# LimpBunion22/VIT-FPGA

Hardware: AMD Instinct MI355X
Metric: images/sec ViT-B/16 224x224, batch 512 per GPU (higher is better)
Workload: dtype bf16; 1 GPU; vit_base 224x224x3 inference, 512 images per GPU resident in HBM, random-init weights (seed 0); global_batch=512, per_gpu_batch=512

## Files before the change

vit-fpga_amd/csrc/gemm_epilogue.h:

```cpp
#pragma once

#include "vh_common.h"

namespace vh {

#ifndef VH_EPI_ABL
#define VH_EPI_ABL 0
#endif
#ifndef VH_EPI_NT
#define VH_EPI_NT 1
#endif
template <typename V>
__device__ __forceinline__ void epi_store(V v, V* p) {
    if constexpr (VH_EPI_NT) __builtin_nontemporal_store(v, p);
    else *p = v;
}

struct EpiArgs {
    const float* bias;
    void* out;
    int M, N;
    const float* aux;
    int aux_i;
    const float* stats;
    void* out16;
    float* partials;
    int64_t prow;
    int lead;
};

constexpr bool epi_has_qgelu(int epi) { return epi == VH_EPI_BIAS_QGELU || epi == VH_EPI_LNFOLD_QGELU; }
constexpr bool epi_has_tgelu(int epi) { return epi == VH_EPI_BIAS_TGELU || epi == VH_EPI_LNFOLD_TGELU; }
constexpr bool epi_has_act(int epi) { return epi == VH_EPI_BIAS_GELU || epi == VH_EPI_LNFOLD_GELU || epi_has_qgelu(epi) || epi_has_tgelu(epi); }
constexpr bool epi_is_lnfold(int epi) {
    return epi == VH_EPI_LNFOLD || epi == VH_EPI_LNFOLD_GELU || epi == VH_EPI_LNFOLD_QGELU || epi == VH_EPI_LNFOLD_TGELU;
}
constexpr bool epi_is_16bit(int epi) { return epi == VH_EPI_BIAS || epi == VH_EPI_LNFOLD || epi_has_act(epi); }

__device__ __forceinline__ float gelu_fast(float v) {
    const float u = fabsf(v);
    const float t = __builtin_amdgcn_rcpf(fmaf(0.2316418882f, u, 1.0f));
    float p = fmaf(0.5307027145f, t, -0.7265760135f);
    p = fmaf(p, t, 0.7107068705f);
    p = fmaf(p, t, -0.142248368f);
    p = fmaf(p, t, 0.127414796f);
    p *= t;
    const float h = p * __builtin_amdgcn_exp2f(v * v * -0.72134752044f);
    return fmaf(-u, h, fmaxf(v, 0.f));
}

typedef __attribute__((ext_vector_type(2))) float f32x2;
template <int DEG> struct GeluW;
template <> struct GeluW<9> { static constexpr float a[10] = {1.111100093e-01f, 5.562581867e-02f, 3.875113651e-02f, 7.441916317e-02f, -2.459328771e-01f,
                                                                1.095633626e+00f, -2.419960260e+00f, 3.303298712e+00f, -2.415727854e+00f, 8.016663194e-01f}; };
template <> struct GeluW<8> { static constexpr float a[9] = {1.111119911e-01f, 5.524744466e-02f, 5.048053339e-02f, -6.402773410e-02f, 5.648611188e-01f,
                                                               -1.549515009e+00f, 2.612281084e+00f, -2.240322828e+00f, 8.585962057e-01f}; };
template <> struct GeluW<6> { static constexpr float a[7] = {1.111383960e-01f, 5.238987878e-02f, 9.770081192e-02f, -3.239865899e-01f, 1.061976552e+00f,
                                                               -1.360716462e+00f, 7.577903271e-01f}; };
__device__ __forceinline__ f32x2 pk_fma_clamp01(f32x2 a, f32x2 b, f32x2 c) {
    f32x2 d;
    asm("v_pk_fma_f32 %0, %1, %2, %3 clamp" : "=v"(d) : "v"(a), "v"(b), "v"(c));
    return d;
}
template <int DEG>
__device__ __forceinline__ f32x4 gelu_poly4(f32x4 v) {
    constexpr const float* a = GeluW<DEG>::a;
    f32x2 x[2] = {f32x2{v[0], v[1]}, f32x2{v[2], v[3]}}, w[2], p[2];
#pragma unroll
    for (int h = 0; h < 2; ++h) w[h] = x[h] * x[h];
#pragma unroll
    for (int h = 0; h < 2; ++h) w[h] = pk_fma_clamp01(w[h], f32x2{-4.938271605e-02f, -4.938271605e-02f}, f32x2{1.f, 1.f});
#pragma unroll
    for (int h = 0; h < 2; ++h) p[h] = __builtin_elementwise_fma(w[h], f32x2{a[DEG], a[DEG]}, f32x2{a[DEG - 1], a[DEG - 1]});
#pragma unroll
    for (int k = DEG - 2; k >= 0; --k)
#pragma unroll
        for (int h = 0; h < 2; ++h) p[h] = __builtin_elementwise_fma(p[h], w[h], f32x2{a[k], a[k]});
#pragma unroll
    for (int h = 0; h < 2; ++h) p[h] = pk_fma_clamp01(x[h], p[h], f32x2{0.5f, 0.5f});
#pragma unroll
    for (int h = 0; h < 2; ++h) x[h] = x[h] * p[h];
    return f32x4{x[0][0], x[0][1], x[1][0], x[1][1]};
}
template <typename T> struct GeluDeg { static constexpr int value = 9; };
template <> struct GeluDeg<BF16> { static constexpr int value = 8; };
template <> struct GeluDeg<E4M3> { static constexpr int value = 6; };

__device__ __forceinline__ f32x4 qgelu4(f32x4 v) {
    constexpr float K = -1.702f * 1.44269504088896341f;
    f32x2 x[2] = {f32x2{v[0], v[1]}, f32x2{v[2], v[3]}}, t[2];
// ... 115 lines not shown
                if constexpr (EPI == VH_EPI_BIAS_F32) *p = v;
                else *p = v + addv[ni];
            }
        }
    }
}

#ifndef VH_EPI_PRIO
#define VH_EPI_PRIO 1
#endif
__device__ __forceinline__ void epi_consts_from_lds(const char* sw, int frow, int fq, f32x4 (&bv)[4], f32x4 (&cv)[4], float2 (&lnst)[8]) {
    const uint32_t la = (uint32_t)(uintptr_t)sw + (uint32_t)((fq * 4) * 4), lr = (uint32_t)(uintptr_t)sw + (uint32_t)(frow * 8);
    asm volatile("ds_read_b128 %0, %8 offset:1024\n\tds_read_b128 %1, %8 offset:1088\n\tds_read_b128 %2, %8 offset:1152\n\tds_read_b128 %3, %8 offset:1216\n\t"
                 "ds_read_b128 %4, %8 offset:1280\n\tds_read_b128 %5, %8 offset:1344\n\tds_read_b128 %6, %8 offset:1408\n\tds_read_b128 %7, %8 offset:1472"
                 : "=&v"(bv[0]), "=&v"(bv[1]), "=&v"(bv[2]), "=&v"(bv[3]), "=&v"(cv[0]), "=&v"(cv[1]), "=&v"(cv[2]), "=&v"(cv[3]) : "v"(la));
    asm volatile("ds_read_b64 %0, %8\n\tds_read_b64 %1, %8 offset:128\n\tds_read_b64 %2, %8 offset:256\n\tds_read_b64 %3, %8 offset:384\n\t"
                 "ds_read_b64 %4, %8 offset:512\n\tds_read_b64 %5, %8 offset:640\n\tds_read_b64 %6, %8 offset:768\n\tds_read_b64 %7, %8 offset:896\n\t"
                 "s_waitcnt lgkmcnt(0)"
                 : "=&v"(lnst[0]), "=&v"(lnst[1]), "=&v"(lnst[2]), "=&v"(lnst[3]), "=&v"(lnst[4]), "=&v"(lnst[5]), "=&v"(lnst[6]), "=&v"(lnst[7]) : "v"(lr));
    asm volatile("" : "+v"(bv[0]), "+v"(bv[1]), "+v"(bv[2]), "+v"(bv[3]), "+v"(cv[0]), "+v"(cv[1]), "+v"(cv[2]), "+v"(cv[3]));
}

template <typename T, int EPI, int MI, int NI, int SMI = MI, bool MFULL = false, bool OTILED = false>
__device__ __forceinline__ void gemm_epilogue_staged(const f32x4 (&acc)[MI][NI], const EpiArgs& e, int m_w, int n_w,
                                                     int lane, char* sw, int prio_grp = -1, bool cpre = false) {
    static_assert(NI == 4, "staged epilogue assumes a 64-column wave tile");
    static_assert(MI % SMI == 0 && SMI % 2 == 0, "slice must divide the wave tile");
    using elem = typename T::elem;
    const int M = e.M, N = e.N;
    const int frow = lane & 15, fq = lane >> 4;
    f32x4 bv[NI], cv[NI];
    float2 lnst[epi_is_lnfold(EPI) ? MI : 1];
    auto consts_from_global = [&]() {
#pragma unroll
        for (int ni = 0; ni < NI; ++ni) {
            bv[ni] = *(const f32x4*)(e.bias + n_w + ni * 16 + fq * 4);
            if constexpr (epi_is_lnfold(EPI)) cv[ni] = *(const f32x4*)(e.aux + n_w + ni * 16 + fq * 4);
            else cv[ni] = f32x4{0.f, 0.f, 0.f, 0.f};
        }
        if constexpr (epi_is_lnfold(EPI)) {
#pragma unroll
            for (int mi = 0; mi < MI; ++mi) {
                int m = m_w + mi * 16 + frow;
                if constexpr (!MFULL) m = m < M ? m : M - 1;
                lnst[mi] = *(const float2*)(e.stats + 2 * (int64_t)m);
            }
        }
    };
    if constexpr (epi_is_lnfold(EPI) && MI == 8) {
        if (cpre) epi_consts_from_lds(sw, frow, fq, bv, cv, lnst);
        else consts_from_global();
    } else {
        consts_from_global();
    }

    if constexpr (epi_is_16bit(EPI) && (VH_EPI_ABL & 64)) {
#pragma unroll
        for (int mi = 0; mi < MI; ++mi)
#pragma unroll
            for (int ni = 0; ni < NI; ++ni) asm volatile("" :: "v"(acc[mi][ni]));
    } else if constexpr (epi_is_16bit(EPI) && epi_has_act(EPI) && MFULL && OTILED) {
        char* const obase = (char*)e.out + ((int64_t)(m_w >> 4) * (N >> 3) + (n_w >> 3) + (fq & 1) * 2 + (fq >> 1)) * 256 + frow * 16;
#pragma unroll
        for (int mi = 0; mi < MI; ++mi) {
            if constexpr (VH_EPI_PRIO == 1) {
                if (prio_grp >= 0 && (mi & 1) == 0) {
                    if (((mi >> 1) + prio_grp) & 1) __builtin_amdgcn_s_setprio(1);
                    else __builtin_amdgcn_s_setprio(0);
                }
            }
            float rstd = 0.f, mr = 0.f;
            if constexpr (epi_is_lnfold(EPI)) { rstd = lnst[mi].y; mr = lnst[mi].x * lnst[mi].y; }
#pragma unroll
            for (int j = 0; j < NI / 2; ++j) {
                const f32x4 v0 = epi_value16<EPI, T>(acc[mi][2 * j], bv[2 * j], cv[2 * j], mr, rstd);
                const f32x4 v1 = epi_value16<EPI, T>(acc[mi][2 * j + 1], bv[2 * j + 1], cv[2 * j + 1], mr, rstd);
                const u32x2 p0 = __builtin_bit_cast(u32x2, pack4<T>(v0[0], v0[1], v0[2], v0[3]));
                const u32x2 p1 = __builtin_bit_cast(u32x2, pack4<T>(v1[0], v1[1], v1[2], v1[3]));
                const auto sx = __builtin_amdgcn_permlane16_swap(p0[0], p1[0], false, false);
                const auto sy = __builtin_amdgcn_permlane16_swap(p0[1], p1[1], false, false);
                epi_store(u32x4{sx[0], sy[0], sx[1], sy[1]}, (u32x4*)(obase + (int64_t)mi * (N >> 3) * 256 + j * 1024));
            }
        }
        if constexpr (VH_EPI_PRIO == 1) { if (prio_grp >= 0) __builtin_amdgcn_s_setprio(0); }
    } else if constexpr (epi_is_16bit(EPI)) {
        const int rr = lane >> 3, pc = lane & 7;
#pragma unroll
        for (int h = 0; h < MI / SMI; ++h) {
            if constexpr (VH_EPI_PRIO == 1) {
                if (prio_grp >= 0) {
                    if ((h + prio_grp) & 1) __builtin_amdgcn_s_setprio(1);
                    else __builtin_amdgcn_s_setprio(0);
                }
            }
#pragma unroll
            for (int mi = 0; mi < SMI; ++mi) {
                if constexpr (VH_EPI_PRIO == 2) {
                    if (prio_grp >= 0) {
                        if ((h * SMI + mi + prio_grp) & 1) __builtin_amdgcn_s_setprio(1);
                        else __builtin_amdgcn_s_setprio(0);
                    }
                }
                const int r = mi * 16 + frow;
                float rstd = 0.f, mr = 0.f;
                if constexpr (epi_is_lnfold(EPI)) {
                    const float2 st = lnst[h * SMI + mi];
// ... 344 lines not shown
```

vit-fpga_amd/csrc/kernels_attn.hip:

```cpp
#include <type_traits>

#include "attn_common.h"

namespace vh {

template <typename T, typename TO = T>
__global__ void __launch_bounds__(1024, 4)
attention_kernel(const typename T::elem* __restrict__ qkv, typename TO::elem* __restrict__ out,
                 int tokens, int heads, int slabs, int ntiles) {
    using elem = typename T::elem;
    using vec8 = typename T::vec8;
    using vec4 = typename T::vec4;
    extern __shared__ __attribute__((aligned(16))) char smem[];
    const int kv_bytes = ntiles * 4096;

    const int lane = threadIdx.x & 63;
    const int wave = __builtin_amdgcn_readfirstlane(threadIdx.x >> 6);
    const int nw = blockDim.x >> 6;
    const int l31 = lane & 31, hl = lane >> 5;
    const int D = heads * 64;
    const int64_t ld = 3 * (int64_t)D;

    const int lr = lane >> 3, pc = lane & 7;
    const int ngroups = ntiles * 4;
// ... 116 lines not shown
        f32x16 s_cur = qk(0);
        for (int kt = 0; kt + 1 < ntiles; ++kt) {
            const VFrag vfr = load_v(kt);
            const f32x16 s_nxt = qk(kt + 1);
            softmax_pv(kt, s_cur, vfr, std::false_type{});
            s_cur = s_nxt;
        }
        {
            const VFrag vfr = load_v(ntiles - 1);
            softmax_pv(ntiles - 1, s_cur, vfr, std::true_type{});
        }

        const float ltot = cross_half_sum(lsum);
        const float inv = 1.0f / ltot;
        const int q = q0 + l31;
        if (q < tokens) {
            typename TO::elem* op = out + ((int64_t)b * tokens + q) * D + h * 64 + 4 * hl;
#pragma unroll
            for (int rg = 0; rg < 4; ++rg) {
                *(typename TO::vec4*)(op + 8 * rg) = pack4<TO>(o0[4 * rg] * inv, o0[4 * rg + 1] * inv, o0[4 * rg + 2] * inv, o0[4 * rg + 3] * inv);
                *(typename TO::vec4*)(op + 32 + 8 * rg) = pack4<TO>(o1[4 * rg] * inv, o1[4 * rg + 1] * inv, o1[4 * rg + 2] * inv, o1[4 * rg + 3] * inv);
            }
        }
    }
}

#ifndef VH_ATTN_ABL
#define VH_ATTN_ABL 0
#endif
__device__ __forceinline__ void ring_dma16(const void* base, uint32_t lane_off, uint32_t lds_addr) {
    asm_lds_dma16(base, lane_off, lds_addr);
}
#ifdef VH_DIAG_STAMPS
__device__ unsigned long long g_attn_diag[1024 * 16 * 16];
__device__ __forceinline__ unsigned long long attn_rt() {
    unsigned long long t;
    asm volatile("s_memrealtime %0\n\ts_waitcnt lgkmcnt(0)" : "=s"(t)::"memory");
    return t;
}
__device__ __forceinline__ unsigned long long attn_ct() {
    unsigned long long t;
    asm volatile("s_memtime %0\n\ts_waitcnt lgkmcnt(0)" : "=s"(t)::"memory");
    return t;
}
#define VH_ATT_T(i) do { __builtin_amdgcn_sched_barrier(0); const unsigned long long n_ = attn_ct(); ph_[i] += n_ - last_; last_ = n_; __builtin_amdgcn_sched_barrier(0); } while (0)
#else
#define VH_ATT_T(i) do { } while (0)
#endif
__device__ __forceinline__ void ring_wait_vm(int n) { wait_vm<40>(n); }
__device__ __forceinline__ void ring_wait_dma() {
    asm volatile("s_waitcnt vmcnt(0)" ::: "memory");
}

template <typename T, typename TO = T, bool QS = false, bool OTILE = false, bool IHM = false>
__global__ void __launch_bounds__(1024, 4)
attention_ring_kernel(const typename T::elem* __restrict__ qkv, typename TO::elem* __restrict__ out,
                      int tokens, int heads, int slabs, int ntiles, int nitems, unsigned int* __restrict__ ticket,
                      unsigned int heads_rcp, int64_t hm_rows) {
    using elem = typename T::elem;
    using vec8 = typename T::vec8;
    using vec4 = typename T::vec4;
    extern __shared__ __attribute__((aligned(16))) char smem[];
    const int G = (tokens + 7) >> 3, G2 = (G + 1) & ~1;
    const int kv_bytes = QS ? G * 1024 : ntiles * 4096;
    const int q_off = kv_bytes + (QS ? G2 * 1024 : kv_bytes);
    const uint32_t lds0 = (uint32_t)(uintptr_t)smem;

    const int lane = threadIdx.x & 63;
    const int wave = __builtin_amdgcn_readfirstlane(threadIdx.x >> 6);
    const int nw = blockDim.x >> 6;
    const int l31 = lane & 31, hl = lane >> 5;
    const int D = heads * 64;
    const int64_t ld = IHM ? 64 : 3 * (int64_t)D;
    const uint32_t koff2 = IHM ? (uint32_t)(hm_rows * D * 2) : (uint32_t)(D * 2);
    auto head_base = [&](int b, int h) {
        if constexpr (IHM) return qkv + ((int64_t)h * hm_rows + (int64_t)b * tokens) * 64;
        else return qkv + (int64_t)b * tokens * ld + h * 64;
    };

    auto kv_base = [&](int item) {
        if (QS) {
            const int b = (heads == 1 ? item : (int)__umulhi((unsigned)item, heads_rcp)), h = item - b * heads;
            return head_base(b, h);
        }
        const int bh = item / slabs;
        const int b = bh / heads, h = bh - b * heads;
        return head_base(b, h);
    };
    auto issue_tile = [&](const elem* base, int t) {
        int ln = lane;
        asm volatile("" : "+v"(ln));
        const int lr_ = ln >> 3, pc_ = ln & 7;
        const int g = 4 * t + wave;
        const int gk = QS && g >= G ? G - 1 : g, gv = QS && g >= G2 ? G2 - 1 : g;
        const int rowk = gk * 8 + lr_, rowv = gv * 8 + lr_;
        const int rk = rowk < tokens ? rowk : tokens - 1;
        const int rv = rowv < tokens ? rowv : tokens - 1;
        const int ck = pc_ ^ ((rowk >> 1) & 7);
        const int cv = pc_ ^ (((rowv >> 1) & 1) << 2);
        const uint32_t ok = (uint32_t)(rk * (int)ld + ck * 8) * 2u + koff2;
        const uint32_t ov = (uint32_t)(rv * (int)ld + cv * 8) * 2u + 2u * koff2;
        ring_dma16(base, ok, lds0 + gk * 1024);
        ring_dma16(base, ov, lds0 + kv_bytes + gv * 1024);
    };
    auto issue_q = [&](const elem* base) {
        int ln = lane;
        asm volatile("" : "+v"(ln));
        const int lr_ = ln >> 3, pc_ = ln & 7;
        for (int j = 0; j < nw; ++j) {
            const int g = 4 * j + wave;
            const int row = g * 8 + lr_;
            const int rsrc = row < tokens ? row : tokens - 1;
            const int ck = pc_ ^ ((row >> 1) & 7);
            ring_dma16(base, (uint32_t)(rsrc * (int)ld + ck * 8) * 2u, lds0 + q_off + g * 1024);
        }
    };
    auto load_q = [&](int item, vec8 (&qf)[4]) {
        const int bh = item / slabs, slab = item - bh * slabs;
        const int b = bh / heads, h = bh - b * heads;
        int qrow = (slab * nw + wave) * 32 + l31;
        qrow = qrow < tokens ? qrow : tokens - 1;
        const elem* qp = head_base(b, h) + (int64_t)qrow * ld + 8 * hl;
        asm volatile("global_load_dwordx4 %0, %4, off\n\tglobal_load_dwordx4 %1, %4, off offset:32\n\t"
                     "global_load_dwordx4 %2, %4, off offset:64\n\tglobal_load_dwordx4 %3, %4, off offset:96"
                     : "=&v"(qf[0]), "=&v"(qf[1]), "=&v"(qf[2]), "=&v"(qf[3]) : "v"(qp) : "memory");
    };

    const int kswz = (l31 >> 1) & 7;
    const int g4 = lane >> 4, i16 = lane & 15, tq = i16 >> 2, tp = i16 & 3;
    const int vrow0 = 4 * (g4 >> 1) + tq;
    const int vcolb = (16 * (g4 & 1) + 4 * tp) * 2;
    const int k0 = l31 * 128 + ((hl ^ kswz) << 4);
    const int vx = ((vrow0 >> 1) & 1) << 6;
    const int v0 = kv_bytes + vrow0 * 128 + (vcolb ^ vx);

    const int stride = (int)gridDim.x;
    int item = blockIdx.x * slabs;
    const elem* cbase = kv_base(item);
    vec8 qf[4];
    if (wave < 4) {
        if (QS) issue_q(cbase);
        for (int t = 0; t < ntiles; ++t) issue_tile(cbase, t);
    }
    if (!QS) load_q(item, qf);
    bool first = true;
    constexpr int NST = 4;
    const int w_top = 2 * (ntiles - 2) + NST, w_t1 = 2 * (ntiles - 3) + NST + 2, w_mid = 2 * ntiles + nw - 4 + NST, w_last = nw + 2 + 2 * (ntiles - 3);
    bool stored = false;

#ifdef VH_DIAG_STAMPS
    const unsigned long long rt0_ = attn_rt();
    unsigned int dbg_[3] = {0xffffffffu, 0xffffffffu, 0xffffffffu};
    int dbg_n_ = 0;
    unsigned long long ph_[10] = {0, 0, 0, 0, 0, 0, 0, 0, 0, 0}, last_ = attn_ct();
#endif
    const bool dyn = QS && ticket != nullptr && nw >= 5;
    const int tk_off = q_off + 4 * nw * 1024;
    unsigned int tkv = 0;
    while (true) {
        const int slab_now = QS ? 0 : item - (item / slabs) * slabs;
        const bool last_slab = QS || slab_now + 1 == slabs;
        int next = QS ? item + stride : (last_slab ? (item / slabs + stride) * slabs : item + 1);
        if (QS && dyn && !first) {
            if (wave == nw - 1) {
                if (stored) asm volatile("s_waitcnt vmcnt(%0)" :: "n"(NST) : "memory");
                else asm volatile("s_waitcnt vmcnt(0)" ::: "memory");
                asm volatile("" : "+v"(tkv));
                if (lane == 0) *(volatile unsigned int __attribute__((address_space(3)))*)(uintptr_t)(lds0 + tk_off) = 2u * (unsigned)stride + tkv;
            }
        }
        const int b = QS ? (heads == 1 ? item : (int)__umulhi((unsigned)item, heads_rcp)) : (item / slabs) / heads;
        const int slab = slab_now;
        const int h = (QS ? item : item / slabs) - b * heads;
        const int q0 = (slab * nw + wave) * 32;

        VH_ATT_T(7);
        if (QS) {
            ring_wait_vm(first ? 0 : w_top);
        } else {
            if (first || !stored) asm volatile("s_waitcnt vmcnt(0)" ::: "memory");
            else asm volatile("s_waitcnt vmcnt(%0)" :: "n"(NST) : "memory");
            asm volatile("" : "+v"(qf[0]), "+v"(qf[1]), "+v"(qf[2]), "+v"(qf[3]));
        }
        VH_ATT_T(0);
        ring_barrier();
        VH_ATT_T(1);
        if (QS && dyn && !first) next = __builtin_amdgcn_readfirstlane(*(volatile const int __attribute__((address_space(3)))*)(uintptr_t)(lds0 + tk_off));
#if defined(VH_DIAG_STAMPS) && defined(VH_ATTN_TKDBG)
        if (QS && dyn && !first) { if (dbg_n_ < 3) dbg_[dbg_n_++] = (unsigned)next; next = item + stride; }
#endif
        const bool has_next = (unsigned)next < (unsigned)nitems;
        const bool refill = has_next && last_slab;
        const elem* nbase = kv_base(has_next ? next : item);
        if (QS && dyn && has_next && wave == nw - 1 && lane == 0) {
            asm_atomic_add_ret_issue(ticket, 1u, tkv);
        }
        if (!(VH_ATTN_ABL & 2) && !first && slab == 0 && wave < 4) issue_tile(cbase, ntiles - 1);
        if (QS) {
            int qa = q_off + wave * 4096 + k0;
            if constexpr (!std::is_same<T, TO>::value) {
                int ln = lane;
                asm volatile("" : "+v"(ln));
                const int r31 = ln & 31;
                qa = q_off + wave * 4096 + r31 * 128 + ((((ln >> 5)) ^ ((r31 >> 1) & 7)) << 4);
            }
#pragma unroll
            for (int ks = 0; ks < 4; ++ks) qf[ks] = *(const vec8*)(smem + (qa ^ (ks << 5)));
        }

        f32x16 o0, o1;
#pragma unroll
        for (int r = 0; r < 16; ++r) { o0[r] = 0.f; o1[r] = 0.f; }
        float negm = 0.f;
        float lsum = 0.f;

        auto qk = [&](int kt, float init) {
            int ka = k0 + kt * 4096;
            if constexpr (!std::is_same<T, TO>::value) asm volatile("" : "+v"(ka));
            vec8 kf[4];
#pragma unroll
            for (int ks = 0; ks < 4; ++ks) {
                if (VH_ATTN_ABL & 32) kf[ks] = qf[ks]; else if (VH_ATTN_ABL & 128) kf[ks] = *(const vec8*)(smem + ((ka ^ (ks << 5)) & 0x3ff0)); else
                kf[ks] = *(const vec8*)(smem + (ka ^ (ks << 5)));
            }
            __builtin_amdgcn_sched_barrier(0);
            typedef float f32x2 __attribute__((ext_vector_type(2)));
            typedef float f32x8 __attribute__((ext_vector_type(8)));
            const f32x2 i2 = {init, init};
            f32x2 p[8];
#pragma unroll
            for (int i = 0; i < 8; ++i) asm volatile("v_mov_b64 %0, %1" : "=v"(p[i]) : "v"(i2));
            const f32x4 q0 = __builtin_shufflevector(p[0], p[1], 0, 1, 2, 3), q1 = __builtin_shufflevector(p[2], p[3], 0, 1, 2, 3);
            const f32x4 q2 = __builtin_shufflevector(p[4], p[5], 0, 1, 2, 3), q3 = __builtin_shufflevector(p[6], p[7], 0, 1, 2, 3);
            const f32x8 h0 = __builtin_shufflevector(q0, q1, 0, 1, 2, 3, 4, 5, 6, 7), h1 = __builtin_shufflevector(q2, q3, 0, 1, 2, 3, 4, 5, 6, 7);
            f32x16 s = __builtin_shufflevector(h0, h1, 0, 1, 2, 3, 4, 5, 6, 7, 8, 9, 10, 11, 12, 13, 14, 15);
#pragma unroll
            for (int ks = 0; ks < 4; ++ks) {
                if (VH_ATTN_ABL & 16) s[ks] += (float)kf[ks][0] * (float)qf[ks][0];
                else s = T::mfma32(kf[ks], qf[ks], s);
            }
            return s;
        };
        struct VFrag { vec8 f[2][2]; };
        auto load_v = [&](int kt) {
            VFrag v;
            if (VH_ATTN_ABL & 32) { for (int ks = 0; ks < 2; ++ks) { v.f[ks][0] = qf[ks]; v.f[ks][1] = qf[ks + 2]; } return v; }
            const char* p0 = smem + (v0 + kt * 4096);
            const char* p1 = smem + ((v0 + kt * 4096) ^ 64);
#pragma unroll
            for (int ks = 0; ks < 2; ++ks) {
                const vec4 a0 = T::tr_read(p0 + ks * 2048), c0 = T::tr_read(p0 + ks * 2048 + 1024);
                const vec4 a1 = T::tr_read(p1 + ks * 2048), c1 = T::tr_read(p1 + ks * 2048 + 1024);
#pragma unroll
                for (int j = 0; j < 4; ++j) { v.f[ks][0][j] = a0[j]; v.f[ks][0][4 + j] = c0[j]; v.f[ks][1][j] = a1[j]; v.f[ks][1][4 + j] = c1[j]; }
            }
            return v;
        };
        auto softmax_pv = [&](int kt, f32x16& s, const VFrag& vfr, auto first_c, auto tail_c) {
            constexpr bool FIRST = decltype(first_c)::value, TAIL = decltype(tail_c)::value;
            int ng = 4;
            if constexpr (TAIL) {
                const int valid = tokens - kt * 32;
                ng = (valid + 7) >> 3;
#pragma unroll
                for (int g = 0; g < 4; ++g)
                    if (g < ng) {
#pragma unroll
                        for (int j = 0; j < 4; ++j)
                            if (8 * g + j + 4 * hl >= valid) s[4 * g + j] = -INFINITY;
                    }
            }
            float mx = -INFINITY;
#pragma unroll
            for (int g = 0; g < 4; ++g)
                if (!TAIL || g < ng) {
#pragma unroll
// ... 96 lines not shown
                    }
                }
            } else {
                const int64_t mrow = (int64_t)b * tokens + (q < tokens ? q : tokens - 1);
                typename TO::elem* const op = OTILE ? out + ((mrow >> 4) * (D >> 4) + h * 4) * 256 + (mrow & 15) * 16 + 8 * hl
                                                    : out + mrow * D + h * 64 + 8 * hl;
#pragma unroll
                for (int db = 0; db < 2; ++db) {
                    const f32x16& o = db ? o1 : o0;
#pragma unroll
                    for (int rg = 0; rg < 4; rg += 2) {
                        const uint32_t ga = pack4<TO>(o[4 * rg] * inv, o[4 * rg + 1] * inv, o[4 * rg + 2] * inv, o[4 * rg + 3] * inv);
                        const uint32_t gb = pack4<TO>(o[4 * rg + 4] * inv, o[4 * rg + 5] * inv, o[4 * rg + 6] * inv, o[4 * rg + 7] * inv);
                        const auto sx = __builtin_amdgcn_permlane32_swap(ga, gb, false, false);
                        if (q < tokens) *(u32x2*)(op + (OTILE ? (2 * db + (rg >> 1)) * 256 : 32 * db + 8 * rg)) = u32x2{sx[0], sx[1]};
                    }
                }
            }
        }
        VH_ATT_T(9);
        if (!has_next) break;
        stored = q0 < tokens;
        item = next;
        cbase = nbase;
        first = false;
    }
#ifdef VH_DIAG_STAMPS
    VH_ATT_T(7);
    if (lane == 0 && blockIdx.x < 1024) {
#pragma unroll
        for (int i = 0; i < 10; ++i) g_attn_diag[((size_t)blockIdx.x * 16 + wave) * 16 + i] = ph_[i];
        unsigned int hw;
        asm volatile("s_getreg_b32 %0, hwreg(HW_REG_HW_ID)" : "=s"(hw));
        unsigned int xcc;
        asm volatile("s_getreg_b32 %0, hwreg(HW_REG_XCC_ID)" : "=s"(xcc));
        g_attn_diag[((size_t)blockIdx.x * 16 + wave) * 16 + 10] = rt0_;
        g_attn_diag[((size_t)blockIdx.x * 16 + wave) * 16 + 11] = attn_rt();
        g_attn_diag[((size_t)blockIdx.x * 16 + wave) * 16 + 12] = ((unsigned long long)xcc << 32) | hw;
        for (int i = 0; i < 3; ++i) g_attn_diag[((size_t)blockIdx.x * 16 + wave) * 16 + 13 + i] = dbg_[i];
    }
#endif
}

#ifdef VH_DIAG_STAMPS
extern "C" int vh_diag_attn_read(unsigned long long* host, int n_words) {
    return (int)hipMemcpyFromSymbol(host, HIP_SYMBOL(g_attn_diag), (size_t)n_words * 8);
}
#endif

size_t attention_lds_bytes(int tokens) { return (size_t)((tokens + 31) / 32) * 8192; }

enum class AttnForm { NONE, ONE_SHOT, RING, RING_QS };
struct AttnPlan { AttnForm form; int slabs, nw; size_t lds; };
static AttnPlan attn_plan(int tokens, bool out_tiled, bool in_head_major) {
    constexpr int kMaxWaves = 16;
    const int ntiles = (tokens + 31) / 32;
    const int slabs = (ntiles + kMaxWaves - 1) / kMaxWaves, nw = (ntiles + slabs - 1) / slabs;
    const size_t one = attention_lds_bytes(tokens);
    if (one > 160 * 1024) return {AttnForm::NONE, slabs, nw, 0};
    const int G = (tokens + 7) / 8, G2 = (G + 1) & ~1;
    const size_t qs_lds = (size_t)(G + G2 + 4 * nw) * 1024 + 16;
    if (slabs == 1 && nw >= 4 && 2 * qs_lds <= 160 * 1024) return {AttnForm::RING_QS, slabs, nw, qs_lds};
    if (ntiles >= 3 && nw >= 4) return {AttnForm::RING, slabs, nw, one};
    if (out_tiled || in_head_major) return {AttnForm::NONE, slabs, nw, 0};
    return {AttnForm::ONE_SHOT, slabs, nw, one};
}
bool attention_tiled_applies(int batch, int tokens, int heads) {
    (void)batch;
    return attn_plan(tokens, true, false).form != AttnForm::NONE && heads % 2 == 0;
}

template <typename T, typename TO = T, bool OTILE = false, bool IHM = false>
static hipError_t launch_attn_t(const void* qkv, int batch, int tokens, int heads, void* out, unsigned int* ticket, hipStream_t s, bool tk_zeroed,
                                int64_t hm_rows = 0) {
    const AttnPlan p = attn_plan(tokens, OTILE, IHM);
    if (p.form == AttnForm::NONE) return hipErrorInvalidValue;
    const int ntiles = (tokens + 31) / 32, slabs = p.slabs, nw = p.nw;
    const int nitems = batch * heads * slabs;
    const int num_cu = device_num_cu();
    if (!num_cu) return hipErrorUnknown;
    if (p.form == AttnForm::RING_QS) {
        auto k = attention_ring_kernel<T, TO, true, OTILE, IHM>;
        static LdsDone lds_done;
        if (hipError_t e = ensure_dynamic_lds((const void*)k, p.lds, lds_done); e != hipSuccess) return e;
        const int grid = nitems < 2 * num_cu ? nitems : 2 * num_cu;
        unsigned int* tk = nw >= 5 && nitems > 2 * grid ? ticket : nullptr;
        if (tk && !tk_zeroed) { if (hipError_t e = hipMemsetAsync(tk, 0, sizeof(unsigned int), s); e != hipSuccess) return e; }
        const unsigned int heads_rcp = (unsigned int)(((1ull << 32) + (unsigned)heads - 1) / (unsigned)heads);
        hipLaunchKernelGGL(k, dim3(grid), dim3(nw * 64), p.lds, s, (const typename T::elem*)qkv, (typename TO::elem*)out,
                           tokens, heads, slabs, ntiles, nitems, tk, heads_rcp, hm_rows);
        return hipGetLastError();
    }
    if (p.form == AttnForm::RING) {
        auto k = attention_ring_kernel<T, TO, false, OTILE, IHM>;
        static LdsDone lds_done;
        if (hipError_t e = ensure_dynamic_lds((const void*)k, p.lds, lds_done); e != hipSuccess) return e;
        const int per_cu = (int)(160 * 1024 / p.lds);
        int grid = num_cu * (per_cu < 1 ? 1 : (per_cu > 2 ? 2 : per_cu));
        if (grid > batch * heads) grid = batch * heads;
        hipLaunchKernelGGL(k, dim3(grid), dim3(nw * 64), p.lds, s, (const typename T::elem*)qkv, (typename TO::elem*)out,
                           tokens, heads, slabs, ntiles, nitems, (unsigned int*)nullptr, 0u, hm_rows);
        return hipGetLastError();
    }
    if constexpr (OTILE || IHM) return hipErrorInvalidValue;
    else {
        auto k = attention_kernel<T, TO>;
        static LdsDone lds_done;
        if (hipError_t e = ensure_dynamic_lds((const void*)k, p.lds, lds_done); e != hipSuccess) return e;
        hipLaunchKernelGGL(k, dim3(nitems), dim3(nw * 64), p.lds, s, (const typename T::elem*)qkv, (typename TO::elem*)out,
                           tokens, heads, slabs, ntiles);
        return hipGetLastError();
    }
}

template <typename T>
__global__ void __launch_bounds__(256)
attention_cls_kernel(const typename T::elem* __restrict__ qkv, typename T::elem* __restrict__ out, int batch, int tokens, int heads) {
    using elem = typename T::elem;
    using vec8 = typename T::vec8;
    constexpr int MAXT = 1024;
    __shared__ float sc[4][MAXT];
    const int lane = threadIdx.x & 63, wv = threadIdx.x >> 6;
    const int item = blockIdx.x * 4 + wv;
    if (item >= batch * heads) return;
    const int b = item / heads, h = item - b * heads;
    const int D = heads * 64;
    const int64_t ld = 3 * (int64_t)D;
    const elem* const base = qkv + (int64_t)b * tokens * ld + h * 64;
    const int g = lane >> 3, c = lane & 7;
    float q[8];
    {
        const vec8 v = *(const vec8*)(base + c * 8);
#pragma unroll
        for (int j = 0; j < 8; ++j) q[j] = (float)v[j];
    }
    float mx = -INFINITY;
    constexpr int U = 4;
    for (int t0 = 0; t0 < tokens; t0 += 8 * U) {
        vec8 v[U];
#pragma unroll
        for (int u = 0; u < U; ++u) {
            const int t = t0 + 8 * u + g;
            v[u] = *(const vec8*)(base + (t < tokens ? t : tokens - 1) * ld + D + c * 8);
        }
#pragma unroll
        for (int u = 0; u < U; ++u) {
            const int t = t0 + 8 * u + g;
// ... 10 lines not shown
#pragma unroll
    for (int o = 32; o > 0; o >>= 1) mx = fmaxf(mx, __shfl_xor(mx, o));
    __builtin_amdgcn_s_waitcnt(0xC07F);
    float sum = 0.f;
    for (int t = lane; t < tokens; t += 64) {
        const float p = __builtin_amdgcn_exp2f(sc[wv][t] - mx);
        sc[wv][t] = p;
        sum += p;
    }
#pragma unroll
    for (int o = 32; o > 0; o >>= 1) sum += __shfl_xor(sum, o);
    __builtin_amdgcn_s_waitcnt(0xC07F);
    float acc[8] = {0.f, 0.f, 0.f, 0.f, 0.f, 0.f, 0.f, 0.f};
    for (int t0 = 0; t0 < tokens; t0 += 8 * U) {
        vec8 v[U];
#pragma unroll
        for (int u = 0; u < U; ++u) {
            const int t = t0 + 8 * u + g;
            v[u] = *(const vec8*)(base + (t < tokens ? t : tokens - 1) * ld + 2 * D + c * 8);
        }
#pragma unroll
        for (int u = 0; u < U; ++u) {
            const int t = t0 + 8 * u + g;
            const float p = t < tokens ? sc[wv][t] : 0.f;
#pragma unroll
            for (int j = 0; j < 8; ++j) acc[j] = fmaf(p, (float)v[u][j], acc[j]);
        }
    }
#pragma unroll
    for (int j = 0; j < 8; ++j) {
        acc[j] += __shfl_xor(acc[j], 8); acc[j] += __shfl_xor(acc[j], 16); acc[j] += __shfl_xor(acc[j], 32);
    }
    if (g == 0) {
        const float r = 1.0f / sum;
        vec8 o;
#pragma unroll
        for (int j = 0; j < 8; ++j) o[j] = (elem)(acc[j] * r);
        *(vec8*)(out + (int64_t)b * D + h * 64 + c * 8) = o;
    }
}
hipError_t launch_attention_cls(const void* qkv16, int batch, int tokens, int heads, void* out16, int dtype, hipStream_t s) {
    if (batch <= 0 || tokens <= 0 || tokens > 1024 || heads <= 0) return hipErrorInvalidValue;
    const dim3 grid((unsigned)((batch * heads + 3) / 4));
    if (dtype == VH_DTYPE_BF16)
        hipLaunchKernelGGL(attention_cls_kernel<BF16>, grid, dim3(256), 0, s, (const BF16::elem*)qkv16, (BF16::elem*)out16, batch, tokens, heads);
    else if (dtype == VH_DTYPE_FP16)
        hipLaunchKernelGGL(attention_cls_kernel<FP16>, grid, dim3(256), 0, s, (const FP16::elem*)qkv16, (FP16::elem*)out16, batch, tokens, heads);
    else
        return hipErrorInvalidValue;
    return hipGetLastError();
}

hipError_t launch_attention(const void* qkv16, int batch, int tokens, int heads, void* out16, int dtype,
                            unsigned int* ticket, hipStream_t s, bool ticket_zeroed, bool out_tiled, int64_t in_hm_rows) {
    if (batch <= 0 || tokens <= 0 || heads <= 0) return hipErrorInvalidValue;
    if (in_hm_rows) {
        if (!out_tiled || in_hm_rows < (int64_t)batch * tokens || in_hm_rows * heads * 64 * 4 >= (1ll << 32)) return hipErrorInvalidValue;
        if (!attention_tiled_applies(batch, tokens, heads)) return hipErrorInvalidValue;
        if (dtype == VH_DTYPE_FP8) return launch_attn_t<BF16, E4M3, true, true>(qkv16, batch, tokens, heads, out16, ticket, s, ticket_zeroed, in_hm_rows);
        return dtype == VH_DTYPE_BF16 ? launch_attn_t<BF16, BF16, true, true>(qkv16, batch, tokens, heads, out16, ticket, s, ticket_zeroed, in_hm_rows)
                                      : launch_attn_t<FP16, FP16, true, true>(qkv16, batch, tokens, heads, out16, ticket, s, ticket_zeroed, in_hm_rows);
    }
    if (out_tiled) {
        if (!attention_tiled_applies(batch, tokens, heads)) return hipErrorInvalidValue;
        if (dtype == VH_DTYPE_FP8) return launch_attn_t<BF16, E4M3, true>(qkv16, batch, tokens, heads, out16, ticket, s, ticket_zeroed);
        return dtype == VH_DTYPE_BF16 ? launch_attn_t<BF16, BF16, true>(qkv16, batch, tokens, heads, out16, ticket, s, ticket_zeroed)
                                      : launch_attn_t<FP16, FP16, true>(qkv16, batch, tokens, heads, out16, ticket, s, ticket_zeroed);
    }
    if (attention_lds_bytes(tokens) > 160 * 1024) return launch_attention_hd(qkv16, batch, tokens, heads, 64, out16, dtype, s);
    if (dtype == VH_DTYPE_FP8) return launch_attn_t<BF16, E4M3>(qkv16, batch, tokens, heads, out16, ticket, s, ticket_zeroed);
    return dtype == VH_DTYPE_BF16 ? launch_attn_t<BF16>(qkv16, batch, tokens, heads, out16, ticket, s, ticket_zeroed)
                                  : launch_attn_t<FP16>(qkv16, batch, tokens, heads, out16, ticket, s, ticket_zeroed);
}

}
```

vit-fpga_amd/csrc/kernels_gemm.hip:

```cpp
#include <cstdio>
#include <cstdlib>

#include "gemm_epilogue.h"
#include "vh_kernels.h"

namespace vh {

template <typename T, int BM, int BN, int WM, int WN, int EPI>
__global__ void __launch_bounds__(WM* WN * 64)
gemm_nt_kernel(const typename T::elem* __restrict__ A, const typename T::elem* __restrict__ W,
               const float* __restrict__ bias, void* __restrict__ outp, int M, int N, int K,
               const float* __restrict__ aux, int aux_i, int tiles_m, int tiles_n, const float* __restrict__ stats,
               void* __restrict__ out16, float* __restrict__ partials, int64_t prow, int lead) {
    using elem = typename T::elem;
    using vec8 = typename T::vec8;
    constexpr int NW = WM * WN;
    constexpr int BK = 64;
    constexpr int ROWS = BM + BN;
    constexpr int STAGE_BYTES = ROWS * 128;
    constexpr int GROUPS_A = BM / 8;
    constexpr int GROUPS = ROWS / 8;
    constexpr int LOADS = GROUPS / NW;
    constexpr int LOADS_A = GROUPS_A / NW;
    constexpr int TM = BM / WM, TN = BN / WN;
// ... 134 lines not shown
    const int64_t t256 = ((M + 255) / 256) * ((N + 255) / 256);
    return t256 >= min_tiles ? gemm_pp_variant(epilogue) : 1;
}

bool gemm_tiled_applies(int64_t M, int N, int K, int dtype) {
    const bool f8 = dtype == VH_DTYPE_FP8;
    const int kt = f8 ? 128 : 64;
    return M > 0 && M % 256 == 0 && N % 256 == 0 && K % kt == 0 && K / kt >= 4 &&
           (f8 ? gemm_pp_variant(VH_EPI_BIAS) : gemm_pick_variant(M, N, VH_EPI_BIAS)) == 6;
}

const char* gemm_check(const GemmArgs& g) {
    const int epi = g.epilogue;
    const bool f8 = g.dtype == VH_DTYPE_FP8;
    const bool act = epi_has_act(epi), fold = epi_is_lnfold(epi), resid = epi == VH_EPI_RESID_LN || epi == VH_EPI_RESID_SPLIT;
    if (f8) {
        if (g.variant != 0 && g.variant != 5 && g.variant != 6 && g.variant != 7) return "gemm_fp8: variant must be 0, 5, 6 or 7";
        if (!g.a || !g.w || !g.wscale || !g.bias || !g.out) return "gemm_fp8: null pointer";
        if (g.M <= 0 || g.N <= 0 || g.K <= 0 || g.K % 128 || g.N % 4) return "gemm_fp8: need K % 128 == 0 and N % 4 == 0";
        if (g.M > 0x7FFFFFFF / 2) return "gemm_fp8: M too large";
        if (!fold && !resid && !act && epi != VH_EPI_BIAS && epi != VH_EPI_BIAS_RESID && epi != VH_EPI_BIAS_F32)
            return "gemm_fp8: epilogue not available";
        if (fold && (!g.aux || !g.stats)) return "gemm_fp8: LNFOLD needs c and stats";
        if (resid && (!g.out16 || !g.partials)) return "gemm_fp8: RESID_* needs out16 and partials";
        if ((resid || (fold && act)) && g.N % 256) return "gemm_fp8: N % 256 != 0";
    } else {
        if (g.M <= 0 || g.N <= 0 || g.K <= 0) return "gemm: empty shape";
        if (g.K % 64) return "gemm: K must be a multiple of 64";
        if (g.N % 4) return "gemm: N must be a multiple of 4";
        if (g.M > 0x7fffffff) return "gemm: M too large";
        if (epi < 0 || epi > VH_EPI_LNFOLD_TGELU || epi == VH_EPI_LNFOLD_QGELU + 1) return "gemm: unknown epilogue";
        if (fold && (!g.stats || !g.aux)) return "gemm: LNFOLD needs stats and c (aux)";
        if (resid && (!g.out16 || !g.partials || g.N % 256)) return "gemm: RESID_LN / RESID_SPLIT need out16, partials and N % 256 == 0";
        if (epi == VH_EPI_PATCH && (!g.aux || g.aux_i <= 0)) return "gemm: EPI_PATCH needs pos-emb and patches/image";
        if ((epi == VH_EPI_PATCH || epi == VH_EPI_PATCH_SPLIT) && (g.lead < 0 || g.lead > 1 + VH_MAX_REGISTERS)) return "gemm: EPI_PATCH* lead rows outside 0..17";
        if (epi == VH_EPI_PATCH_SPLIT && (!g.aux || g.aux_i <= 0 || !g.out16 || !g.partials || g.N % 256 || g.prow < 0))
            return "gemm: EPI_PATCH_SPLIT needs pos-emb, patches/image, the lo plane, partials and N % 256 == 0";
        if (g.dtype != VH_DTYPE_BF16 && g.dtype != VH_DTYPE_FP16) return "gemm: dtype";
        if (g.variant < 0 || g.variant > 7) return "gemm: variant";
        if (g.variant == 3 || g.variant == 4) return "gemm: variants 3/4 (BK=32 pipeline) were removed";
        if (!g.a || !g.w || !g.bias || !g.out) return "gemm: null pointer";
    }
    if (g.out_tiled || g.ab_tiled) {
        if (g.out_tiled && g.ab_tiled) return "gemm_layout: out_tiled and ab_tiled exclude each other";
        if (g.variant != 6) return "gemm_layout: the tiled layouts exist in the persistent form only (variant 6)";
        if (g.tile_begin || g.tile_count) return "gemm_layout: a tile range excludes the tiled layouts";
        if (g.M % 256 || g.N % 256) return "gemm_layout: the tiled layouts need M % 256 == 0 and N % 256 == 0";
        const bool four = fold && !(f8 && act);
        if (g.K / (f8 ? 128 : 64) < (four ? 4 : 2))
            return four ? "gemm_layout: the tiled layouts need at least 4 K-tiles with this epilogue"
                        : "gemm_layout: the tiled layouts need at least 2 K-tiles with this epilogue";
        if (g.out_tiled && !(act || epi == VH_EPI_LNFOLD || (!f8 && epi == VH_EPI_BIAS)))
            return "gemm_layout: out_tiled goes with the activation epilogues (tiled) or LNFOLD / 16-bit BIAS (head-major)";
        if (g.ab_tiled && !(epi == VH_EPI_RESID_SPLIT || (!f8 && epi == VH_EPI_BIAS))) return "gemm_layout: ab_tiled goes with RESID_SPLIT or 16-bit BIAS";
    }
    if (g.tile_begin < 0 || g.tile_count < 0) return "gemm_layout: negative tile range";
    if (g.tile_begin || g.tile_count) {
        if (g.variant != 5 && g.variant != 7) return "gemm_layout: tile ranges exist in variants 5 and 7 only";
        if (!g.tile_count) return "gemm_layout: tile_begin != 0 needs tile_count > 0";
        const int64_t tiles = ((g.M + 255) / 256) * ((g.N + 255) / 256);
        if ((int64_t)g.tile_begin + g.tile_count > tiles) {
            static thread_local char text[64];
            snprintf(text, sizeof text, "gemm_layout: tile range beyond the %lld tiles", (long long)tiles);
            return text;
        }
    }
    return nullptr;
}

hipError_t launch_gemm_fp8(const GemmArgs& g, hipStream_t s);

hipError_t launch_gemm(const GemmArgs& g, hipStream_t s) {
    if (gemm_check(g)) return hipErrorInvalidValue;
    if (g.dtype == VH_DTYPE_FP8) return launch_gemm_fp8(g, s);
    const int variant = g.variant ? g.variant : gemm_pick_variant(g.M, g.N, g.epilogue);
    return g.dtype == VH_DTYPE_BF16 ? launch_epi<BF16>(g, variant, s) : launch_epi<FP16>(g, variant, s);
}

}
```

vit-fpga_amd/csrc/kernels_gemm5.hip:

```cpp
#include <cstdlib>
#include <type_traits>

#include "gemm_epilogue.h"
#include "vh_kernels.h"

#ifndef VH_PP_SMI
#define VH_PP_SMI 2
#endif

namespace vh {

#ifndef VH_MAIN_ABL
#define VH_MAIN_ABL 0
#endif
#ifndef VH_PP_CPRE
#define VH_PP_CPRE 1
#endif
constexpr int kAblHalf = (VH_MAIN_ABL & 64) ? 1 : 0;
constexpr int kWPieces = kAblHalf ? 2 : 4;
#ifdef VH_DIAG_STAMPS
#ifndef VH_DIAG_KT
#define VH_DIAG_KT -1
#endif
#ifndef VH_DIAG_REC_IT
// ... 412 lines not shown
    if (env >= 0) return env > 0 && env < tiles_n ? env : 0;
    if (tiles_n < 6) return 0;
    if (tiles_n % 4 == 0) return 4;
    if (tiles_n % 3 == 0) return 3;
    return 4;
}

#ifdef VH_DIAG_STAMPS
struct DiagRec { int64_t M; int N, K, epi, f8, grid, variant; };
static unsigned long long* g_diag_buf = nullptr;
static int g_diag_slots = 0, g_diag_max_wgs = 0;
static long long g_diag_count = 0;
static DiagRec g_diag_rec[1024];
static unsigned long long* diag_next(const GemmArgs& g, int epi, bool f8, int grid, int variant) {
    if (!g_diag_buf || grid > g_diag_max_wgs) return nullptr;
    const int slot = (int)(g_diag_count % g_diag_slots);
    g_diag_rec[slot] = DiagRec{g.M, g.N, g.K, epi, f8 ? 1 : 0, grid, variant};
    ++g_diag_count;
    return g_diag_buf + (size_t)slot * g_diag_max_wgs * 128;
}
#define VH_STAMP_ARG(g, epi, f8, grid, variant) , diag_next(g, epi, f8, grid, variant)
#else
#define VH_STAMP_ARG(g, epi, f8, grid, variant)
#endif

template <typename T, int EPI, bool F8, bool PERSIST, int AST, bool OT = false, bool AT = false>
static hipError_t launch_pp_one(const GemmArgs& g, int grid, int tiles_m, int tiles_n, hipStream_t s) {
    constexpr size_t lds = (AST == 3 || PERSIST) ? 163840 : 131072;
    auto k = gemm_nt_pp_kernel<T, EPI, PERSIST, F8, AST, OT, AT>;
    static LdsDone lds_done;
    if (hipError_t e = ensure_dynamic_lds((const void*)k, lds, lds_done); e != hipSuccess) return e;
    hipLaunchKernelGGL(k, dim3(grid), dim3(512), lds, s, g.a, g.w, g.bias, g.out, (int)g.M, g.N, g.K, g.aux, g.aux_i, tiles_m,
                       tiles_n, g.stats, g.out16, g.partials, PERSIST ? 0 : g.tile_begin, (g.tile_count || g.tile_begin) ? 0 : gemm_super_columns(tiles_n),
                       F8 ? g.wscale : (const float*)nullptr, gemm_prow(g), g.lead
                       VH_STAMP_ARG(g, EPI, F8, grid, PERSIST ? 6 : (AST == 3 ? 7 : 5)));
    return hipGetLastError();
}

template <typename T, int EPI, bool F8>
static hipError_t launch_pp(const GemmArgs& g, int mode, hipStream_t s) {
    if constexpr (EPI == VH_EPI_PATCH) { if (mode == 1) mode = 0; }
    const int tiles_m = (int)((g.M + 255) / 256), tiles_n = (g.N + 255) / 256;
    const int ntiles = g.tile_count > 0 ? g.tile_count : tiles_m * tiles_n;
    if (mode == 2) return launch_pp_one<T, EPI, F8, false, 3>(g, ntiles, tiles_m, tiles_n, s);
    if constexpr (EPI != VH_EPI_PATCH) {
        const int full_m = (int)(g.M / 256);
        const int nk = g.K / (F8 ? 128 : 64);
        if (mode == 1 && (g.N % 256 != 0 || full_m == 0 || nk < (pp_uses_cpre<EPI, F8>() ? 4 : 2))) mode = 0;
        if (mode == 1 && full_m != tiles_m && g.variant != 6) mode = 0;
        if (mode == 1) {
            const int num_cu = device_num_cu();
            if (!num_cu) return hipErrorUnknown;
            const int nfull = full_m * tiles_n, grid = nfull < num_cu ? nfull : num_cu;
            if constexpr (epi_has_act(EPI) || EPI == VH_EPI_LNFOLD || (!F8 && EPI == VH_EPI_BIAS)) {
                if (g.out_tiled) return launch_pp_one<T, EPI, F8, true, 2, true, false>(g, grid, full_m, tiles_n, s);
            }
            if constexpr (F8 ? EPI == VH_EPI_RESID_SPLIT : (EPI == VH_EPI_RESID_SPLIT || EPI == VH_EPI_BIAS)) {
                if (g.ab_tiled) return launch_pp_one<T, EPI, F8, true, 2, false, true>(g, grid, full_m, tiles_n, s);
            }
            if (hipError_t e = launch_pp_one<T, EPI, F8, true, 2>(g, grid, full_m, tiles_n, s); e != hipSuccess) return e;
            if (full_m == tiles_m) return hipSuccess;
            GemmArgs tail = g;
            tail.tile_begin = nfull;
            tail.tile_count = tiles_n;
            return launch_pp_one<T, EPI, F8, false, 2>(tail, tiles_n, tiles_m, tiles_n, s);
        }
    }
    return launch_pp_one<T, EPI, F8, false, 2>(g, ntiles, tiles_m, tiles_n, s);
}

template <typename T, int EPI>
hipError_t launch_gemm_pingpong(const GemmArgs& g, int mode, hipStream_t s) {
    return launch_pp<T, EPI, false>(g, mode, s);
}

#define VH_INST(T)                                                                                     \
    template hipError_t launch_gemm_pingpong<T, VH_EPI_BIAS>(const GemmArgs&, int, hipStream_t);       \
    template hipError_t launch_gemm_pingpong<T, VH_EPI_BIAS_GELU>(const GemmArgs&, int, hipStream_t);  \
    template hipError_t launch_gemm_pingpong<T, VH_EPI_BIAS_RESID>(const GemmArgs&, int, hipStream_t); \
    template hipError_t launch_gemm_pingpong<T, VH_EPI_BIAS_F32>(const GemmArgs&, int, hipStream_t);   \
    template hipError_t launch_gemm_pingpong<T, VH_EPI_PATCH>(const GemmArgs&, int, hipStream_t);       \
    template hipError_t launch_gemm_pingpong<T, VH_EPI_LNFOLD>(const GemmArgs&, int, hipStream_t);      \
    template hipError_t launch_gemm_pingpong<T, VH_EPI_LNFOLD_GELU>(const GemmArgs&, int, hipStream_t); \
    template hipError_t launch_gemm_pingpong<T, VH_EPI_RESID_LN>(const GemmArgs&, int, hipStream_t);   \
    template hipError_t launch_gemm_pingpong<T, VH_EPI_RESID_SPLIT>(const GemmArgs&, int, hipStream_t); \
    template hipError_t launch_gemm_pingpong<T, VH_EPI_PATCH_SPLIT>(const GemmArgs&, int, hipStream_t); \
    template hipError_t launch_gemm_pingpong<T, VH_EPI_BIAS_QGELU>(const GemmArgs&, int, hipStream_t);  \
    template hipError_t launch_gemm_pingpong<T, VH_EPI_LNFOLD_QGELU>(const GemmArgs&, int, hipStream_t); \
    template hipError_t launch_gemm_pingpong<T, VH_EPI_BIAS_TGELU>(const GemmArgs&, int, hipStream_t);  \
    template hipError_t launch_gemm_pingpong<T, VH_EPI_LNFOLD_TGELU>(const GemmArgs&, int, hipStream_t);
VH_INST(BF16)
VH_INST(FP16)

hipError_t launch_gemm_fp8(const GemmArgs& g, hipStream_t s) {
    const int v = g.variant ? g.variant : gemm_pp_variant(g.epilogue);
    const int mode = v == 7 ? 2 : (v == 6 ? 1 : 0);
    switch (g.epilogue) {
        case VH_EPI_BIAS: return launch_pp<BF16, VH_EPI_BIAS, true>(g, mode, s);
        case VH_EPI_BIAS_GELU: return launch_pp<BF16, VH_EPI_BIAS_GELU, true>(g, mode, s);
        case VH_EPI_BIAS_QGELU: return launch_pp<BF16, VH_EPI_BIAS_QGELU, true>(g, mode, s);
        case VH_EPI_BIAS_TGELU: return launch_pp<BF16, VH_EPI_BIAS_TGELU, true>(g, mode, s);
        case VH_EPI_BIAS_RESID: return launch_pp<BF16, VH_EPI_BIAS_RESID, true>(g, mode, s);
        case VH_EPI_BIAS_F32: return launch_pp<BF16, VH_EPI_BIAS_F32, true>(g, mode, s);
        case VH_EPI_LNFOLD: return launch_pp<BF16, VH_EPI_LNFOLD, true>(g, mode, s);
        case VH_EPI_LNFOLD_GELU: return launch_pp<BF16, VH_EPI_LNFOLD_GELU, true>(g, mode, s);
        case VH_EPI_LNFOLD_QGELU: return launch_pp<BF16, VH_EPI_LNFOLD_QGELU, true>(g, mode, s);
// ... 33 lines not shown
```

vit-fpga_amd/csrc/vh_kernels.h:

```cpp
#pragma once

#include <atomic>
#include <cstdlib>
#include <vector>

#include "vh_common.h"

namespace vh {

struct GemmArgs {
    const void* a;
    const void* w;
    const float* bias;
    void* out;
    int64_t M;
    int N, K;
    int epilogue;
    const float* aux;
    int aux_i;
    int dtype;
    int variant;
    const float* stats = nullptr;
    void* out16 = nullptr;
    float* partials = nullptr;
    const float* wscale = nullptr;
    int tile_begin = 0, tile_count = 0;
    int64_t prow = 0;
    int out_tiled = 0, ab_tiled = 0;
    int lead = 1;
};
bool gemm_tiled_applies(int64_t M, int N, int K, int dtype);
hipError_t launch_cast_tiled_w(const float* w, int rows, int cols, void* w16, int dtype, hipStream_t stream);
hipError_t launch_tile_bytes(const void* w8, int rows, int cols, void* out, hipStream_t stream);

inline int64_t gemm_prow(const GemmArgs& g) {
    if (g.epilogue != VH_EPI_PATCH_SPLIT) return g.M;
    return g.prow > 0 ? g.prow : (g.M / g.aux_i) * (int64_t)(g.aux_i + g.lead);
}

hipError_t launch_gemm(const GemmArgs& g, hipStream_t stream);
const char* gemm_check(const GemmArgs& g);
int gemm_pick_variant(int64_t M, int N, int epilogue);
int gemm_pp_variant(int epilogue);

hipError_t launch_layernorm(const float* x, int64_t rows, int dim, int64_t row_stride,
                            const float* gamma, const float* beta, float eps, void* out16,
                            int dtype, hipStream_t stream);
hipError_t launch_head_f32(const float* y, const float* w, const float* bias, float* out, int batch, int classes, int dim,
                           hipStream_t stream);
hipError_t launch_head_f32_groups(const float* y, int64_t ldy, int64_t y_step, const float* w, const float* bias, float* out, int64_t ldo,
                                  const float* add, int batch, int classes, int dim, int groups, hipStream_t stream);
hipError_t launch_act_f32(float* x, int64_t n, int act, hipStream_t stream);
constexpr float kAttnQScale = 0.125f * 1.4426950408889634f;
hipError_t launch_attention(const void* qkv16, int batch, int tokens, int heads, void* out16,
                            int dtype, unsigned int* ticket, hipStream_t stream, bool ticket_zeroed = false, bool out_tiled = false,
                            int64_t in_hm_rows = 0);
bool attention_tiled_applies(int batch, int tokens, int heads);
hipError_t launch_attention_cls(const void* qkv16, int batch, int tokens, int heads, void* out16, int dtype, hipStream_t stream);
size_t attention_lds_bytes(int tokens);
constexpr int kAttnStreamMaxTokens = 4097;
constexpr int kAttnHdMaxWidth = 2048;
bool attention_hd_supported(int head_dim);
hipError_t launch_attention_hd(const void* qkv16, int batch, int tokens, int heads, int head_dim, void* out16, int dtype,
                               hipStream_t stream);
constexpr int kAttnMapsMaxQueries = 17;
const char* attention_probs_check(int64_t in_hm_rows, int batch, int tokens, int heads, int head_dim, int Q, int dtype);
hipError_t launch_attention_probs(const void* qkv16, int64_t in_hm_rows, int batch, int tokens, int heads, int head_dim, int Q, int dtype,
                                  float* probs, hipStream_t stream);
const char* rope_check(const void* qkv16, int dtype, int batch, int tokens, int heads, int head_dim, int lead, int64_t hm_rows,
                       const float* cos_t, const float* sin_t);
hipError_t launch_rope(void* qkv16, int dtype, int batch, int tokens, int heads, int head_dim, int lead, int64_t hm_rows, const float* cos_t,
                       const float* sin_t, hipStream_t stream);
const char* attention_readout_check(int batch, int heads, int Q, int tokens, int lead, int elem, int keys);
hipError_t launch_attention_readout(const float* store, int batch, int heads, int Q, int tokens, int lead, int elem, int keys, void* probs_out,
                                    void* mean_out, hipStream_t stream);
inline float attention_q_scale(int head_dim) {
    return head_dim == 64 ? kAttnQScale : (float)(1.4426950408889634 / __builtin_sqrt((double)head_dim));
}
hipError_t launch_im2col(const float* in_nhwc, int batch, int image, int patch, int channels, int kpad,
                         void* out16, int dtype, hipStream_t stream);
constexpr int kMaxChannels = 64;
hipError_t launch_im2col_u8(const uint8_t* in_nhwc, int batch, int image, int patch, int channels, int kpad,
                            const float* scale, const float* shift, void* out16, int dtype, hipStream_t stream);
hipError_t launch_im2col_tensor(const void* in, int elem, int layout, int batch, int image, int patch, int channels, int kpad,
                                const float* scale, const float* shift, void* out16, int dtype, hipStream_t stream);
constexpr int kResizeMaxTaps = 65, kResizeMaxScale = 32, kResizeMaxSide = 8192;
constexpr int kResizeLdsFloats = 16384;
constexpr int kResizeFrameWords = 16;
int resize_axis_table(int n_in, double lo, double hi, int n_out, int32_t* first, int32_t* count, float* weights, int max_taps);
const char* resize_plan_build(const vh_frame* desc, int batch, int channels, int S, size_t nbytes, bool base_aligned4,
                              std::vector<uint32_t>* words, int* max_tiles);
hipError_t launch_resize_u8(const uint8_t* frames, const uint32_t* plan_dev, int batch, int channels, int S, int max_tiles,
                            uint8_t* out_u8, hipStream_t stream);
constexpr int kResizeNv12FrameWords = 24;
int resize_axis_table_over(int n_in, double lo, double hi, double over, int n_out, int32_t* first, int32_t* count, float* weights,
                           int max_taps);
const char* resize_plan_build_nv12(const vh_frame_nv12* desc, int batch, int S, size_t nbytes, unsigned base_mod4, int chroma_site,
                                   int sample_bytes, std::vector<uint32_t>* words, int* max_tiles);
int yuv_matrix(int standard, int full_range, float m[12]);
const char* resize_plan_build_yuv(const vh_frame_yuv* desc, int batch, int S, size_t nbytes, bool base_even, int chroma_site, int sample_bytes,
                                  std::vector<uint32_t>* words, int* max_tiles);
int yuv_matrix16(int standard, int full_range, int bits, int msb_aligned, float m[12]);
hipError_t launch_resize_yuv_any(bool planar, bool wide, const uint8_t* frames, const uint32_t* plan_dev, int batch, int S, int max_tiles,
                                 const float* m12_host, uint8_t* out_u8, hipStream_t stream);
const char* resize_plan_build_yuy2(const vh_frame_yuy2* desc, int batch, int S, size_t nbytes, unsigned base_mod8, int chroma_site,
                                   int sample_bytes, std::vector<uint32_t>* words, int* max_tiles);
hipError_t launch_resize_yuy2(bool wide, const uint8_t* frames, const uint32_t* plan_dev, int batch, int S, int max_tiles,
                              const float* m12_host, uint8_t* out_u8, hipStream_t stream);
const char* resize_plan_build_bgra(const vh_frame_bgra* desc, int batch, int S, size_t nbytes, unsigned base_mod8, int sample_bytes,
                                   std::vector<uint32_t>* words, int* max_tiles);
// ... 115 lines not shown
```

vit-fpga_amd/csrc/vithip_api.hip:

```cpp
#include <dlfcn.h>

#include <chrono>
#include <cmath>
#include <condition_variable>
#include <cstdarg>
#include <cstdio>
#include <cstdlib>
#include <cstring>
#include <functional>
#include <memory>
#include <mutex>
#include <string>
#include <thread>
#include <vector>

#include "vh_kernels.h"

using namespace vh;

namespace {

thread_local std::string g_err;

int fail(std::string* ctx_err, int code, const char* fmt, ...) {
// ... 164 lines not shown
}

struct ImgIn {
    const void* p;
    int kind = VH_ELEM_F32;
    int layout = VH_LAYOUT_NHWC;
    bool u8() const { return kind == VH_ELEM_U8; }
    bool nhwc_f32() const { return kind == VH_ELEM_F32 && layout == VH_LAYOUT_NHWC; }
    size_t elem() const { return kind == VH_ELEM_F32 ? 4 : kind == VH_ELEM_U8 ? 1 : 2; }
    ImgIn skip(size_t elements) const { return ImgIn{(const char*)p + elements * elem(), kind, layout}; }
    bool operator==(const ImgIn& o) const { return p == o.p && kind == o.kind && layout == o.layout; }
};
constexpr int kU8 = VH_ELEM_U8;

struct ActSet {
    char* base = nullptr;
    unsigned int* tickets = nullptr;
    float* x = nullptr;
    void* xn16 = nullptr;
    void* xlo16 = nullptr;
    void* qkv16 = nullptr;
    void* att16 = nullptr;
    void* h16 = nullptr;
    void* col16 = nullptr;
    float* clsn32 = nullptr;
    float* pool32 = nullptr;
    float* stats = nullptr;
    float* partials = nullptr;
    float *mapz32 = nullptr, *maph32 = nullptr, *mapa32 = nullptr;
};
struct ActSetLayout { size_t x, xn, qkv, att, h, col, cls, pool, st, pt, xlo, tk, mz, mh, ma, bytes; };

struct vh_ctx {
    vh_config cfg;
    int device;
    Layout L;
    hipStream_t stream = nullptr;
    static constexpr int kMaxStreams = 4;
    hipStream_t xstream[kMaxStreams - 1] = {nullptr, nullptr, nullptr};
    hipEvent_t ev_fork = nullptr, ev_join[kMaxStreams - 1] = {nullptr, nullptr, nullptr};
    int nstreams = 1;
    hipEvent_t ev0 = nullptr, ev1 = nullptr;
    bool weights_ready = false;
    int run_layers = -1;
    char* blob = nullptr;
    float* params = nullptr;
    char* w16 = nullptr;
    void* wp16 = nullptr;
    std::vector<void*> wqkv16, wo16, w1_16, w2_16;
    std::vector<void*> w2t_16, wot_16;
    bool h_tiled = false;
    bool att_tiled = true;
    bool qkv_hm = true;
    bool weights_ready_tiled = false;
    float* bqkv = nullptr;
    bool fp8 = false;
    int dt16 = VH_DTYPE_BF16;
    std::vector<float*> sqkv, so, s1, s2;
    bool ln_fold = false;
    float* fold_cd = nullptr;
    bool split = false;
    bool cls_tail = false;
    int head_dim = 64;
    float q_scale = kAttnQScale;
    bool ln_fold_cfg = false, split_cfg = false;
    unsigned int* guard_dev = nullptr;
    float* guard_host = nullptr;
    float guard_thresh = 0.5f;
    bool guard_auto = false, guard_tripped = false;
    char* arena = nullptr;
    ActSet act[2];
    ActSetLayout act_layout{};
    int last_set = 0;
    hipStream_t stream2 = nullptr;
    hipEvent_t ev_fork2 = nullptr, ev_join2 = nullptr, ev_head[2] = {nullptr, nullptr};
    int inflight_max = 2, ring_flip = 0;
    bool s2_open = false;
    float* in_dev = nullptr;
    float in_scale[kMaxChannels], in_shift[kMaxChannels];
    float* logits_dev = nullptr;
    uint8_t* rz_u8 = nullptr;
    uint32_t *rz_plan_dev = nullptr, *rz_plan_host = nullptr;
    size_t rz_plan_dev_cap = 0, rz_plan_host_cap = 0;
    uint8_t* rz_frames = nullptr;
    size_t rz_frames_cap = 0;
    std::vector<uint32_t> rz_words;
    struct FrameColour { float m[12]; int site = VH_CHROMA_LEFT; };
    FrameColour colour[2];
    int64_t last_us = 0;
    bool timed = false;
    int last_batch = 0;
    int feat_layers[VH_MAX_FEATURE_LAYERS] = {0}, feat_n = 0;
    char* feat_store = nullptr;
    size_t feat_slot = 0;
    int cap_layers[VH_MAX_FEATURE_LAYERS] = {0}, cap_n = 0, cap_nl = -1, cap_form = VH_FEAT_FORM_F32;
    int attn_layers[VH_MAX_ATTENTION_LAYERS] = {0}, attn_n = 0, attn_q = 0, attn_mode = VH_ATTN_Q_CLS;
    char* attn_store = nullptr;
    size_t attn_slot = 0;
    int acap_layers[VH_MAX_ATTENTION_LAYERS] = {0}, acap_n = 0, acap_nl = -1;
    struct RingSlot {
        float *h_in = nullptr, *h_out = nullptr, *d_in = nullptr, *d_out = nullptr;
        hipEvent_t in_done = nullptr, fwd_done = nullptr, out_done = nullptr;
        int batch = 0;
        uint32_t* h_plan = nullptr;
        size_t plan_cap = 0;
    };
    std::vector<RingSlot> ring;
    enum RingKind { RING_F32, RING_U8, RING_FRAMES, RING_TENSOR };
    RingKind ring_kind = RING_F32;
    int ring_elem = VH_ELEM_F32, ring_layout = VH_LAYOUT_NHWC;
    size_t ring_slot_bytes = 0;
    hipStream_t copy_in = nullptr, copy_out = nullptr;
    int ring_batch = 0, ring_wr = 0, ring_rd = 0, ring_used = 0;
    bool last_h_tiled = false;
    bool last_qkv_hm = false;
    int num_cu = 256;
    bool use_graph = false;
    struct GraphEntry { ImgIn in; float* out; int batch; hipGraph_t graph; hipGraphExec_t exec; };
    std::vector<GraphEntry> graphs;
    std::vector<int> graph_warm;
    int timing_stage = -1;
    std::vector<hipEvent_t> tev;
    size_t tev_used = 0;
    bool step_timing = false;
    std::vector<hipEvent_t> sev;
    size_t sev_used = 0;
    std::string err;
};

struct vh_filter {
    int device, height, width, kind;
    struct Slot {
        uint8_t *h_in = nullptr, *h_out = nullptr, *d_in = nullptr, *d_out = nullptr;
        hipEvent_t in_done = nullptr, k_done = nullptr, out_done = nullptr;
    };
    std::vector<Slot> slot;
    hipStream_t copy_in = nullptr, compute = nullptr, copy_out = nullptr;
    int wr = 0, rd = 0, used = 0;
    std::string err;
};

struct vh_mlp {
    int device, n_ins, n_layers, activation;
    std::vector<int> npl;
    size_t n_params = 0, n_neurons = 0;
    int widest = 0, max_vec = 0;
    hipStream_t stream = nullptr;
    float *params = nullptr, *bias = nullptr, *buf0 = nullptr, *buf1 = nullptr;
    bool loaded = false;
    int64_t last_us = 0;
    int n_sets = 0;
    float *set_ins = nullptr, *set_outs = nullptr, *tz = nullptr, *ta = nullptr, *td = nullptr, *terr = nullptr;
    int64_t last_gradient_us = 0;
    std::string err;
};

namespace {

size_t align_up(size_t v, size_t a) { return (v + a - 1) / a * a; }

int set_device(std::string* err, int device) {
    int n = 0;
    hipError_t e = hipGetDeviceCount(&n);
    if (e != hipSuccess || n <= 0) return fail(err, VH_ERR_NO_DEVICE, "no HIP device visible (%s)", hipGetErrorString(e));
    if (device < 0 || device >= n) return fail(err, VH_ERR_INVALID, "device %d out of range (0..%d)", device, n - 1);
    HIPCHK(err, hipSetDevice(device));
    return VH_OK;
}
// ... 233 lines not shown
    const bool pre_ln = (f.flags & VH_FLAG_PRE_LN) != 0;
    const bool quick = (f.flags & VH_FLAG_QUICK_GELU) != 0, tanh_gelu = (f.flags & VH_FLAG_TANH_GELU) != 0;
    const int epi_fc1 = quick ? VH_EPI_LNFOLD_QGELU : tanh_gelu ? VH_EPI_LNFOLD_TGELU : VH_EPI_LNFOLD_GELU;
    const int epi_fc1_plain = quick ? VH_EPI_BIAS_QGELU : tanh_gelu ? VH_EPI_BIAS_TGELU : VH_EPI_BIAS_GELU;
    const bool patch_split = c->split && !c->fp8 && nl > 0 && !pre_ln;
    if ((rc = tmark(ST_IM2COL))) return rc;
    if (in.layout == VH_LAYOUT_NHWC && in.u8())
        HIPCHK(&c->err, launch_im2col_u8((const uint8_t*)in.p, batch, f.image_size, f.patch_size, f.channels, L.KPA, c->in_scale, c->in_shift,
                                         col16, dt16, s));
    else if (in.nhwc_f32())
        HIPCHK(&c->err, launch_im2col((const float*)in.p, batch, f.image_size, f.patch_size, f.channels, L.KPA, col16, dt16, s));
    else
        HIPCHK(&c->err, launch_im2col_tensor(in.p, in.kind, in.layout, batch, f.image_size, f.patch_size, f.channels, L.KPA, c->in_scale,
                                             c->in_shift, col16, dt16, s));
    if ((rc = tmark(ST_IM2COL))) return rc;
    if ((rc = mark(ST_IM2COL))) return rc;
    if (patch_split) {
        GemmArgs g = gemm_args(dt16, col16, c->wp16, P + L.patch_b, xn16, (int64_t)batch * L.NP, D, L.KPA, VH_EPI_PATCH_SPLIT, pos_p, L.NP);
        g.out16 = xlo16;
        g.prow = rows_g;
        g.lead = L.lead;
        if ((rc = stage(ST_PATCH, [&] { return launch_gemm(g, s); }))) return rc;
        if ((rc = stage(ST_CLS, [&] {
                 return launch_lead_rows_split(xn16, xlo16, partials_p, rows_g, cls_p, pos_p, P + L.reg, L.lead, batch, T, D, dt16, s);
             })))
            return rc;
        HIPCHK(&c->err, launch_finalize_stats(partials_p, D / 64, rows_g, D, f.ln_eps, stats_p, s, rows, c->guard_dev, amax_guard));
        if ((rc = mark(ST_LNSTATS))) return rc;
    } else {
        GemmArgs g = gemm_args(dt16, col16, c->wp16, P + L.patch_b, x, (int64_t)batch * L.NP, D, L.KPA, VH_EPI_PATCH, pos_p, L.NP);
        g.lead = L.lead;
        if ((rc = stage(ST_PATCH, [&] { return launch_gemm(g, s); }))) return rc;
        if ((rc = stage(ST_CLS, [&] { return launch_lead_rows(x, cls_p, pos_p, P + L.reg, L.lead, batch, T, D, s); }))) return rc;
        if (pre_ln) {
            const bool fold0 = c->ln_fold && nl > 0;
            if ((rc = stage(ST_PRELN, [&] {
                     return launch_pre_layernorm(x, fold0 ? rows_g : rows, D, P + L.prew, P + L.preb, f.ln_eps, fold0 && c->split ? nullptr : x,
                                                 fold0 ? xn16 : nullptr, fold0 && c->split ? xlo16 : nullptr, fold0 ? stats_p : nullptr, op_dt, s,
                                                 rows, fold0 ? c->guard_dev : nullptr, fold0 ? amax_guard : nullptr);
                 })))
                return rc;
        } else if (c->ln_fold && nl > 0) {
            if (c->split) HIPCHK(&c->err, launch_rowstats_split(x, rows_g, D, f.ln_eps, xn16, xlo16, stats_p, op_dt, s, rows, amax_guard));
            else HIPCHK(&c->err, launch_rowstats_cast(x, rows_g, D, f.ln_eps, xn16, stats_p, op_dt, s, rows, amax_guard));
            HIPCHK(&c->err, launch_ln_guard(stats_p, rows, c->guard_dev, s));
            if ((rc = mark(ST_LNSTATS))) return rc;
        }
    }
    const bool hd64 = c->head_dim == 64;
    const bool tail = c->cls_tail && hd64 && c->ln_fold && c->split && !c->fp8 && nl == f.layers && c->run_layers < 0 && T <= 1024 &&
                      (size_t)L.NP * L.KPA * esz >= 2 * ((size_t)D * esz + 256);
    const bool h_tiled = c->h_tiled && c->split && c->weights_ready_tiled && gemm_tiled_applies(rows_g, M, D, op_dt) && gemm_tiled_applies(rows_g, D, M, op_dt);
    const bool att_tiled = hd64 && h_tiled && c->att_tiled && gemm_tiled_applies(rows_g, D, D, op_dt) && attention_tiled_applies(batch, T, f.heads) && !tail;
    const bool qkv_hm = c->qkv_hm && att_tiled && gemm_tiled_applies(rows_g, 3 * D, D, op_dt);
    c->last_h_tiled = h_tiled && nl > 0 && c->ln_fold;
    c->last_qkv_hm = qkv_hm && nl > 0 && c->ln_fold;
    for (int l = 0; l < nl && c->ln_fold; ++l) {
        const LayerOff& o = L.layer[l];
        const float* cd = c->fold_cd + (size_t)l * (6 * D + 2 * M);
        const int nblk = D / 64;
        const float *sq = c->fp8 ? c->sqkv[l] : nullptr, *so = c->fp8 ? c->so[l] : nullptr;
        const float *s1 = c->fp8 ? c->s1[l] : nullptr, *s2 = c->fp8 ? c->s2[l] : nullptr;
        GemmArgs gq = gemm_args(op_dt, xn16, c->wqkv16[l], cd + 3 * D, qkv16, rows_g, 3 * D, D, VH_EPI_LNFOLD, cd);
        gq.wscale = sq;
        set_tiled(gq, qkv_hm, false);
        if ((rc = stage(ST_QKV, [&] { return launch_gemm(gq, s); }))) return rc;
        if ((rc = rope(qkv_hm ? (int64_t)rows_g : 0))) return rc;
        if ((rc = capture_attention(l, qkv_hm ? (int64_t)rows_g : 0))) return rc;
        if (tail && l + 1 == nl) {
            char* const hc = col16;
            char* const lc = col16 + (((size_t)batch * D * esz + 255) & ~(size_t)255);
            HIPCHK(&c->err, launch_attention_cls(qkv16, batch, T, f.heads, att16, dt16, s));
            if ((rc = mark(ST_ATTN))) return rc;
            HIPCHK(&c->err, hipMemcpy2DAsync(hc, (size_t)D * esz, xn16, (size_t)T * D * esz, (size_t)D * esz, batch, hipMemcpyDeviceToDevice, s));
            HIPCHK(&c->err, hipMemcpy2DAsync(lc, (size_t)D, xlo16, (size_t)T * D, (size_t)D, batch, hipMemcpyDeviceToDevice, s));
            GemmArgs gp = gemm_args(op_dt, att16, c->wo16[l], P + o.ob, hc, batch, D, D, VH_EPI_RESID_SPLIT);
            gp.out16 = lc;
            HIPCHK(&c->err, launch_gemm(gp, s));
            if ((rc = mark(ST_PROJ))) return rc;
            HIPCHK(&c->err, launch_finalize_stats(partials_p, nblk, batch, D, f.ln_eps, stats_p, s, batch, c->guard_dev));
            if ((rc = mark(ST_LNSTATS))) return rc;
            const GemmArgs g1 = gemm_args(op_dt, hc, c->w1_16[l], cd + 6 * D + M, h16, batch, M, D, epi_fc1, cd + 6 * D);
            HIPCHK(&c->err, launch_gemm(g1, s));
            if ((rc = mark(ST_FC1))) return rc;
            GemmArgs g2 = gemm_args(op_dt, h16, c->w2_16[l], P + o.f2b, hc, batch, D, M, VH_EPI_RESID_SPLIT);
            g2.out16 = lc;
            HIPCHK(&c->err, launch_gemm(g2, s));
            if ((rc = mark(ST_FC2))) return rc;
            if (head_wait) HIPCHK(&c->err, hipStreamWaitEvent(s, head_wait, 0));
            HIPCHK(&c->err, launch_layernorm_split(hc, lc, batch, D, D, P + L.lnfw, P + L.lnfb, f.ln_eps, clsn32, dt16, s));
            if ((rc = mark(ST_LNF))) return rc;
            HIPCHK(&c->err, launch_head_f32(clsn32, P + L.headw, P + L.headb, logits, batch, f.classes, D, s));
            if ((rc = mark(ST_HEAD))) return rc;
            c->last_batch = batch;
            return VH_OK;
        }
        if ((rc = stage(ST_ATTN, [&] {
                 return hd64 ? launch_attention(qkv16, batch, T, f.heads, att16, op_dt, tickets_part + l, s, true, att_tiled, qkv_hm ? (int64_t)rows_g : 0)
                             : launch_attention_hd(qkv16, batch, T, f.heads, c->head_dim, att16, op_dt, s);
             })))
            return rc;
        GemmArgs go = gemm_args(op_dt, att16, att_tiled ? c->wot_16[l] : c->wo16[l], P + o.ob, c->split ? (void*)xn16 : x, rows_g, D, D,
                                c->split ? VH_EPI_RESID_SPLIT : VH_EPI_RESID_LN);
        go.out16 = c->split ? xlo16 : xn16;
        go.wscale = so;
        set_tiled(go, false, att_tiled);
        if ((rc = stage(ST_PROJ, [&] { return launch_gemm(go, s); }))) return rc;
        HIPCHK(&c->err, launch_finalize_stats(partials_p, nblk, rows_g, D, f.ln_eps, stats_p, s, rows, c->guard_dev, amax_guard));
        if ((rc = mark(ST_LNSTATS))) return rc;
        GemmArgs g1 = gemm_args(op_dt, xn16, c->w1_16[l], cd + 6 * D + M, h16, rows_g, M, D, epi_fc1, cd + 6 * D);
        g1.wscale = s1;
        set_tiled(g1, h_tiled, false);
        if ((rc = stage(ST_FC1, [&] { return launch_gemm(g1, s); }))) return rc;
        GemmArgs g2 = gemm_args(op_dt, h16, h_tiled ? c->w2t_16[l] : c->w2_16[l], P + o.f2b, c->split ? (void*)xn16 : x, rows_g, D, M,
                                c->split ? VH_EPI_RESID_SPLIT : (l + 1 < nl ? VH_EPI_RESID_LN : VH_EPI_BIAS_RESID));
        g2.out16 = c->split ? xlo16 : xn16;
        g2.wscale = s2;
        set_tiled(g2, false, h_tiled);
        if ((rc = stage(ST_FC2, [&] { return launch_gemm(g2, s); }))) return rc;
        if ((rc = capture(l))) return rc;
        if (l + 1 < nl) {
            HIPCHK(&c->err, launch_finalize_stats(partials_p, nblk, rows_g, D, f.ln_eps, stats_p, s, rows, c->guard_dev, amax_guard));
            if ((rc = mark(ST_LNSTATS))) return rc;
        }
    }
    const bool plain = !c->ln_fold;
    auto ln_rows = [&](const float* w, const float* b) { return launch_layernorm(x, rows, D, D, w, b, f.ln_eps, xn16, op_dt, s); };
    auto resid_gemm_ln = [&](const void* a, const void* w, const float* bias, const float* scale, int K, const float* lnw,
                             const float* lnb, int st_gemm) -> int {
        GemmArgs g = gemm_args(op_dt, a, w, bias, x, rows, D, K, VH_EPI_BIAS_RESID);
        g.wscale = scale;
        if (int r = stage(st_gemm, [&] { return launch_gemm(g, s); })) return r;
        return lnw ? stage(ST_LN, [&] { return ln_rows(lnw, lnb); }) : VH_OK;
    };
    if (plain && nl > 0) {
        const LayerOff& o0 = L.layer[0];
        if ((rc = stage(ST_LN, [&] { return ln_rows(P + o0.ln1w, P + o0.ln1b); }))) return rc;
    }
    for (int l = 0; l < nl && plain; ++l) {
        const LayerOff& o = L.layer[l];
        const float *sq = c->fp8 ? c->sqkv[l] : nullptr, *so = c->fp8 ? c->so[l] : nullptr;
        const float *s1 = c->fp8 ? c->s1[l] : nullptr, *s2 = c->fp8 ? c->s2[l] : nullptr;
        GemmArgs gq = gemm_args(op_dt, xn16, c->wqkv16[l], c->bqkv + (size_t)l * 3 * D, qkv16, rows, 3 * D, D, VH_EPI_BIAS);
        gq.wscale = sq;
        if ((rc = stage(ST_QKV, [&] { return launch_gemm(gq, s); }))) return rc;
        if ((rc = rope(0))) return rc;
        if ((rc = capture_attention(l, 0))) return rc;
        if ((rc = stage(ST_ATTN, [&] {
                 return hd64 ? launch_attention(qkv16, batch, T, f.heads, att16, op_dt, tickets_part + l, s, true)
                             : launch_attention_hd(qkv16, batch, T, f.heads, c->head_dim, att16, op_dt, s);
             })))
// ... 530 lines not shown
    }
    c->num_cu = prop.multiProcessorCount;
    {
        const char* e = getenv("VH_GRAPH");
        c->use_graph = e && e[0] == '1';
    }
    CK(hipEventCreate(&c->ev0));
    CK(hipEventCreate(&c->ev1));
    CK(hipMalloc((void**)&c->blob, sizeof(BlobHeader) + 4 * L.total));
    c->params = (float*)(c->blob + sizeof(BlobHeader));
    size_t w16_bytes = 0;
    auto carve16 = [&](size_t elems) { size_t o = w16_bytes; w16_bytes += align_up(elems * 2, 256); return o; };
    const size_t o_wp = carve16(D * L.KPA);
    std::vector<size_t> o_qkv(cfg->layers), o_o(cfg->layers), o_1(cfg->layers), o_2(cfg->layers), o_2t(cfg->layers);
    const bool want_tiled_any = D % 256 == 0 && M % 256 == 0 && !(getenv("VH_H_TILED") && getenv("VH_H_TILED")[0] == '0');
    const bool want_tiled = cfg->dtype != VH_DTYPE_FP8 && want_tiled_any;
    const bool want_tiled8 = cfg->dtype == VH_DTYPE_FP8 && want_tiled_any;
    for (int l = 0; l < cfg->layers; ++l) {
        o_qkv[l] = carve16(3 * D * D); o_o[l] = carve16(D * D); o_1[l] = carve16(M * D); o_2[l] = carve16(D * M);
        o_2t[l] = want_tiled ? carve16(D * M) : want_tiled8 ? carve16((D * M + 1) / 2) : 0;
    }
    std::vector<size_t> o_ot(cfg->layers);
    for (int l = 0; l < cfg->layers; ++l) o_ot[l] = want_tiled ? carve16(D * D) : want_tiled8 ? carve16((D * D + 1) / 2) : 0;
    const size_t o_bqkv = w16_bytes;
    w16_bytes += align_up((size_t)cfg->layers * 3 * D * 4, 256);
    {
        const bool eligible = (cfg->dim % 256 == 0) && (cfg->mlp_dim % 256 == 0);
        bool want = true;
        if (cfg->flags & VH_FLAG_LN_FOLD_OFF) want = false;
        else if (!(cfg->flags & VH_FLAG_LN_FOLD_ON)) { const char* e = getenv("VH_LN_FOLD"); if (e) want = e[0] == '1'; }
        c->ln_fold = eligible && want;
        c->guard_auto = c->ln_fold && !(cfg->flags & (VH_FLAG_LN_FOLD_ON | VH_FLAG_LN_FOLD_OFF)) && !getenv("VH_LN_FOLD");
        if (const char* e = getenv("VH_LN_GUARD")) { const float t = (float)atof(e); if (t > 0.f) c->guard_thresh = t; }
    }
    c->fp8 = cfg->dtype == VH_DTYPE_FP8;
    c->dt16 = c->fp8 ? VH_DTYPE_BF16 : cfg->dtype;
    for (int i = 0; i < kMaxChannels; ++i) {
        c->in_scale[i] = i < cfg->channels ? 1.0f / 255.0f : 0.f;
        c->in_shift[i] = 0.f;
    }
    yuv_matrix(VH_YUV_BT709, 0, c->colour[0].m);
    yuv_matrix16(VH_YUV_BT709, 0, 10, 1, c->colour[1].m);
    {
        const char* e = getenv("VH_RESID_SPLIT");
        c->split = c->ln_fold && !(e && e[0] == '0');
        c->ln_fold_cfg = c->ln_fold;
        c->split_cfg = c->split;
        c->cls_tail = (cfg->flags & VH_FLAG_CLS_TAIL) != 0;
        c->head_dim = cfg->dim / cfg->heads;
        c->q_scale = attention_q_scale(c->head_dim);
        c->h_tiled = want_tiled || want_tiled8;
        { const char* e = getenv("VH_ATT_TILED"); c->att_tiled = !(e && e[0] == '0'); }
        { const char* e = getenv("VH_QKV_HM"); c->qkv_hm = !(e && e[0] == '0'); }
    }
    CK(hipHostMalloc((void**)&c->guard_host, 64, hipHostMallocDefault));
    *c->guard_host = 0.f;
    const size_t o_cd = w16_bytes;
    w16_bytes += align_up((size_t)cfg->layers * (6 * D + 2 * M) * 4, 256);
    const size_t o_sc = w16_bytes, sc_per_layer = 5 * D + M;
    if (c->fp8) w16_bytes += align_up((size_t)cfg->layers * sc_per_layer * 4, 256);
    CK(hipMalloc((void**)&c->w16, w16_bytes));
    c->wp16 = c->w16 + o_wp; c->bqkv = (float*)(c->w16 + o_bqkv);
    c->fold_cd = (float*)(c->w16 + o_cd);
    for (int l = 0; l < cfg->layers; ++l) {
        c->wqkv16.push_back(c->w16 + o_qkv[l]); c->wo16.push_back(c->w16 + o_o[l]);
        c->w1_16.push_back(c->w16 + o_1[l]); c->w2_16.push_back(c->w16 + o_2[l]);
        c->w2t_16.push_back(want_tiled || want_tiled8 ? c->w16 + o_2t[l] : nullptr);
        c->wot_16.push_back(want_tiled || want_tiled8 ? c->w16 + o_ot[l] : nullptr);
        if (c->fp8) {
            float* sc = (float*)(c->w16 + o_sc) + (size_t)l * sc_per_layer;
            c->sqkv.push_back(sc); c->so.push_back(sc + 3 * D); c->s1.push_back(sc + 4 * D); c->s2.push_back(sc + 4 * D + M);
        }
    }
    size_t a = 0;
    auto carve = [&](size_t bytes) { size_t o = a; a += align_up(bytes, 256); return o; };
    const size_t rows_p = rows + 256;
    ActSetLayout& o = c->act_layout;
    o.x = carve(rows_p * D * 4); o.xn = carve(rows_p * D * 2); o.qkv = carve(rows_p * 3 * D * 2);
    o.att = carve(rows_p * D * 2); o.h = carve(rows_p * M * 2); o.col = carve(B * L.NP * (size_t)L.KPA * 2);
    o.cls = carve(B * 2 * D * 4); o.pool = carve(B * D * 4);
    o.st = carve(rows_p * 2 * 4); o.pt = carve((D / 64 + 1) * rows_p * 2 * 4);
    o.xlo = carve(rows_p * D * 2);
    o.tk = carve(B * 4 * (size_t)(cfg->layers > 0 ? cfg->layers : 1));
    o.mz = L.map ? carve(B * (size_t)cfg->heads * D * 4) : 0; o.mh = L.map ? carve(B * (M > D ? M : D) * 4) : 0;
    o.ma = L.map ? carve(B * 2 * D * 4) : 0;
    o.bytes = a;
    const size_t o_in = carve(B * (size_t)cfg->image_size * cfg->image_size * cfg->channels * 4), o_lg = carve(B * C * 4),
                 o_gd = carve(256);
    CK(hipMalloc((void**)&c->arena, a));
    c->guard_dev = (unsigned int*)(c->arena + o_gd);
    CK(hipMemsetAsync(c->guard_dev, 0, 256, c->stream));
    bind_set(c->act[0], c->arena, o, L.map);
    c->in_dev = (float*)(c->arena + o_in); c->logits_dev = (float*)(c->arena + o_lg);
#undef CK
    *out = c;
    return VH_OK;
}

int vh_destroy(vh_ctx* c) {
    if (!c) return VH_OK;
    hipSetDevice(c->device);
    vh_ring_destroy(c);
    if (c->stream) sync_compute(c);
    drop_graphs(c);
    if (c->guard_host) hipHostFree(c->guard_host);
    if (c->rz_plan_host) hipHostFree(c->rz_plan_host);
// ... 832 lines not shown
    if (c->last_batch <= 0) return fail(&c->err, VH_ERR_STATE, "no forward has run");
    HIPCHK(&c->err, hipSetDevice(c->device));
    HIPCHK(&c->err, sync_compute(c));
    const size_t D = c->cfg.dim;
    if (what == 0) {
        const size_t n = (size_t)c->last_batch * c->L.T * D;
        if (n_floats != n) return fail(&c->err, VH_ERR_INVALID, "expected %zu floats", n);
        const int nl = (c->run_layers < 0 || c->run_layers > c->cfg.layers) ? c->cfg.layers : c->run_layers;
        if (c->split && nl > 0) {
            auto f = [&](uint16_t b, int dt) {
                if (dt == VH_DTYPE_BF16) { uint32_t u = (uint32_t)b << 16; float v; memcpy(&v, &u, 4); return v; }
                _Float16 hv; memcpy(&hv, &b, 2); return (float)hv;
            };
            auto g = [&](uint8_t b) {
                const int e = (b >> 3) & 15, m = b & 7;
                float v = e ? ldexpf(1.f + m / 8.f, e - 7) : ldexpf(m / 8.f, -6);
                return (b & 0x80) ? -v : v;
            };
            if (c->fp8) {
                std::vector<uint8_t> hi(n);
                std::vector<uint16_t> lo(n);
                HIPCHK(&c->err, hipMemcpy(hi.data(), c->act[c->last_set].xn16, n, hipMemcpyDeviceToHost));
                HIPCHK(&c->err, hipMemcpy(lo.data(), c->act[c->last_set].xlo16, n * 2, hipMemcpyDeviceToHost));
                for (size_t i = 0; i < n; ++i) host_out[i] = g(hi[i]) + f(lo[i], VH_DTYPE_BF16);
                return VH_OK;
            }
            std::vector<uint16_t> hi(n);
            std::vector<uint8_t> lo(n);
            HIPCHK(&c->err, hipMemcpy(hi.data(), c->act[c->last_set].xn16, n * 2, hipMemcpyDeviceToHost));
            HIPCHK(&c->err, hipMemcpy(lo.data(), c->act[c->last_set].xlo16, n, hipMemcpyDeviceToHost));
            const float inv = c->dt16 == VH_DTYPE_BF16 ? 1.f / 32.f : 1.f / 256.f;
            for (size_t i = 0; i < n; ++i) host_out[i] = f(hi[i], c->dt16) + g(lo[i]) * inv;
            return VH_OK;
        }
        HIPCHK(&c->err, hipMemcpy(host_out, c->act[c->last_set].x, n * 4, hipMemcpyDeviceToHost));
        return VH_OK;
    }
    if (what == 1) {
        const size_t n = (size_t)c->last_batch * c->L.HW;
        if (n_floats != n) return fail(&c->err, VH_ERR_INVALID, "expected %zu floats", n);
        HIPCHK(&c->err, hipMemcpy(host_out, c->act[c->last_set].clsn32, n * 4, hipMemcpyDeviceToHost));
        return VH_OK;
    }
    if (what == 3) {
        if (n_floats != 1) return fail(&c->err, VH_ERR_INVALID, "expected 1 float");
        host_out[0] = c->last_h_tiled ? 1.f : 0.f;
        return VH_OK;
    }
    if (what == 4) {
        if (n_floats != 1) return fail(&c->err, VH_ERR_INVALID, "expected 1 float");
        host_out[0] = c->last_qkv_hm ? 1.f : 0.f;
        return VH_OK;
    }
    return fail(&c->err, VH_ERR_INVALID, "unknown tap %d", what);
}

int vh_debug_set_layers(vh_ctx* c, int n_layers) {
    if (!c) return fail(nullptr, VH_ERR_INVALID, "null context");
    c->run_layers = n_layers;
    if (c->stream) sync_compute(c);
    drop_graphs(c);
    return VH_OK;
}

static int features_check_call(vh_ctx* c, const vh_features* f, bool device) {
    if (!c) return fail(nullptr, VH_ERR_INVALID, "read_features: null context");
    if (!f) return fail(&c->err, VH_ERR_INVALID, "read_features: null descriptor");
    if (!f->cls && !f->patch && !f->mean) return fail(&c->err, VH_ERR_INVALID, "read_features: no output requested (cls, patch and mean are all NULL)");
    if (f->elem != VH_ELEM_F32 && f->elem != VH_ELEM_F16 && f->elem != VH_ELEM_BF16)
        return fail(&c->err, VH_ERR_INVALID, "read_features: elem %d is not VH_ELEM_F32, VH_ELEM_F16 or VH_ELEM_BF16", f->elem);
    if (f->norm != VH_FEAT_NORM && f->norm != VH_FEAT_RAW) return fail(&c->err, VH_ERR_INVALID, "read_features: norm %d is not VH_FEAT_NORM (0) or VH_FEAT_RAW (1)", f->norm);
    if (device && (((uintptr_t)f->cls | (uintptr_t)f->patch | (uintptr_t)f->mean) & 15))
        return fail(&c->err, VH_ERR_INVALID, "read_features: a device output pointer is not 16-byte aligned (cls %p, patch %p, mean %p)", f->cls, f->patch, f->mean);
    if (c->cfg.flags & VH_FLAG_CLS_TAIL)
        return fail(&c->err, VH_ERR_UNSUPPORTED, "read_features: a VH_FLAG_CLS_TAIL context's last layer updates the class-token rows only");
    if (f->cls && !c->L.ncls) return fail(&c->err, VH_ERR_UNSUPPORTED, "read_features: cls on a context without a class token (VH_FLAG_NO_CLS)");
    if (!c->ring.empty()) return fail(&c->err, VH_ERR_STATE, "read_features: a ring exists on this context (its forwards belong to slots); vh_ring_destroy first");
    if (c->last_batch <= 0) return fail(&c->err, VH_ERR_STATE, "read_features: no forward has run");
    return VH_OK;
}
struct FeatSource { const void* hi; const void* lo; int form; bool head_cls; };
static FeatSource features_live(const vh_ctx* c) {
    const vh_config& g = c->cfg;
    const int nl = (c->run_layers < 0 || c->run_layers > g.layers) ? g.layers : c->run_layers;
    const bool planes = c->split && nl > 0;
    const ActSet& A = c->act[c->last_set];
    return FeatSource{planes ? (const void*)A.xn16 : (const void*)A.x, planes ? A.xlo16 : nullptr,
                      planes ? (c->fp8 ? VH_DTYPE_FP8 : c->dt16) : VH_FEAT_FORM_F32, c->L.pool == VH_POOL_CLS};
}
static int features_enqueue(vh_ctx* c, const vh_layer_features& f, const FeatSource& src, const char* who) {
    const vh_config& g = c->cfg;
    const bool norm = f.norm == VH_FEAT_NORM;
    FeatureArgs a{};
    a.hi = src.hi; a.lo = src.lo; a.form = src.form;
    a.batch = c->last_batch; a.tokens = c->L.T; a.lead = c->L.lead; a.dim = g.dim;
    a.gamma = c->params + c->L.lnfw; a.beta = c->params + c->L.lnfb; a.eps = g.ln_eps;
    a.elem = f.elem; a.norm = f.norm;
    const bool copy_cls = norm && src.head_cls;
    a.cls = copy_cls ? nullptr : f.cls;
    a.patch = f.patch; a.mean = f.mean; a.stats = c->act[c->last_set].stats;
    a.reg = f.reg; a.patch_layout = f.patch_layout;
    a.no_cls = c->L.ncls ? 0 : 1;
    if (a.cls || a.patch || a.mean || a.reg) {
        if (const char* why = features_check(a)) return fail(&c->err, VH_ERR_INVALID, "%s: %s", who, why);
        HIPCHK(&c->err, launch_token_features(a, c->stream));
    }
// ... 264 lines not shown
    if (int rc = attention_check_call(c, f, false, &slot)) return rc;
    HIPCHK(&c->err, hipSetDevice(c->device));
    const size_t es = f->elem == VH_ELEM_F32 ? 4 : 2, B = c->last_batch, Q = c->attn_q;
    const size_t K = f->keys == VH_ATTN_KEYS_PATCH ? c->L.NP : c->L.T;
    const size_t n_probs = B * c->cfg.heads * Q * K * es, n_mean = B * Q * K * es;
    const size_t cap = ((size_t)c->cfg.max_batch * c->L.T + 256) * 3 * c->cfg.dim * 2;
    vh_attention_maps d = *f;
    size_t at = 0;
    if (f->probs) { d.probs = (char*)c->act[c->last_set].qkv16 + at; at += align_up(n_probs, 256); }
    if (f->head_mean) { d.head_mean = (char*)c->act[c->last_set].qkv16 + at; at += align_up(n_mean, 256); }
    if (at > cap) return fail(&c->err, VH_ERR_STATE, "read_attention: staging needs %zu bytes, the scratch holds %zu", at, cap);
    if (int rc = attention_enqueue(c, d, slot)) return rc;
    if (f->probs) HIPCHK(&c->err, hipMemcpyAsync(f->probs, d.probs, n_probs, hipMemcpyDeviceToHost, c->stream));
    if (f->head_mean) HIPCHK(&c->err, hipMemcpyAsync(f->head_mean, d.head_mean, n_mean, hipMemcpyDeviceToHost, c->stream));
    HIPCHK(&c->err, sync_compute(c));
    return VH_OK;
}

#define OPCHK(expr) do { hipError_t e_ = (expr); if (e_ != hipSuccess) return fail(nullptr, VH_ERR_HIP, "%s failed: %s", #expr, hipGetErrorString(e_)); } while (0)

constexpr unsigned kEpiPlain8 = 1u << VH_EPI_BIAS | 1u << VH_EPI_BIAS_GELU | 1u << VH_EPI_BIAS_QGELU | 1u << VH_EPI_BIAS_TGELU | 1u << VH_EPI_BIAS_RESID | 1u << VH_EPI_BIAS_F32;
constexpr unsigned kEpiFold8 = 1u << VH_EPI_LNFOLD | 1u << VH_EPI_LNFOLD_GELU | 1u << VH_EPI_LNFOLD_QGELU | 1u << VH_EPI_LNFOLD_TGELU | 1u << VH_EPI_RESID_LN | 1u << VH_EPI_RESID_SPLIT;
static int op_gemm_run(const char* tag, const GemmArgs& g, unsigned offered8, void* stream) {
    const bool f8 = g.dtype == VH_DTYPE_FP8;
    GemmArgs h = g;
    if (f8 && !offered8) h.dtype = -1;
    const bool lacks = f8 && offered8 && (g.epilogue < 0 || g.epilogue > VH_EPI_LNFOLD_TGELU || !(offered8 >> g.epilogue & 1));
    if (lacks) { h.epilogue = VH_EPI_BIAS; h.out_tiled = h.ab_tiled = h.tile_begin = h.tile_count = 0; }
    if (const char* why = gemm_check(h))
        return f8 && offered8 ? fail(nullptr, VH_ERR_INVALID, "%s%s", tag, strchr(why, ':')) : fail(nullptr, VH_ERR_INVALID, "%s", why);
    if (lacks) return fail(nullptr, VH_ERR_UNSUPPORTED, "%s: epilogue %d not available", tag, g.epilogue);
    hipError_t e = launch_gemm(g, (hipStream_t)stream);
    if (e == hipSuccess) e = hipStreamSynchronize((hipStream_t)stream);
    if (e != hipSuccess) return fail(nullptr, e == hipErrorInvalidValue ? VH_ERR_INVALID : VH_ERR_HIP, "%s failed: %s", tag, hipGetErrorString(e));
    return VH_OK;
}
int vh_op_gemm(const void* a, const void* w, const float* bias, void* out, int64_t M, int N, int K, int epi,
               const float* aux, int aux_i, int dtype, int variant, void* stream) {
    const GemmArgs g{a, w, bias, out, M, N, K, epi, aux, aux_i, dtype, variant};
    return op_gemm_run("gemm", g, 0, stream);
}
int vh_op_gemm_ex(const void* a, const void* w, const float* bias, void* out, int64_t M, int N, int K, int epi,
                  const float* aux, int aux_i, const float* stats, void* out16, float* partials, int dtype, int variant,
                  void* stream) {
    GemmArgs g{a, w, bias, out, M, N, K, epi, aux, aux_i, dtype, variant};
    g.stats = stats; g.out16 = out16; g.partials = partials;
    return op_gemm_run("gemm_ex", g, 0, stream);
}
int vh_op_gemm_layout(const void* a, const void* w, const float* bias, void* out, int64_t M, int N, int K, int epi,
                      const float* aux, int aux_i, const float* stats, void* out16, float* partials, int dtype, int variant,
                      int out_tiled, int ab_tiled, int tile_begin, int tile_count, void* stream) {
    GemmArgs g{a, w, bias, out, M, N, K, epi, aux, aux_i, dtype, variant};
    g.stats = stats; g.out16 = out16; g.partials = partials;
    g.out_tiled = out_tiled; g.ab_tiled = ab_tiled; g.tile_begin = tile_begin; g.tile_count = tile_count;
    return op_gemm_run("gemm_layout", g, 0, stream);
}
int vh_op_gemm_lead(const void* a, const void* w, const float* bias, void* out, int64_t M, int N, int K, int epi, const float* aux,
                    int aux_i, int lead, void* out16, float* partials, int64_t prow, int dtype, int variant, void* stream) {
    if (epi != VH_EPI_PATCH && epi != VH_EPI_PATCH_SPLIT) return fail(nullptr, VH_ERR_INVALID, "gemm_lead: epilogue must be VH_EPI_PATCH or VH_EPI_PATCH_SPLIT");
    if (aux_i > 0 && M % aux_i) return fail(nullptr, VH_ERR_INVALID, "gemm_lead: M must be a whole number of images (M %% aux_i == 0)");
    GemmArgs g{a, w, bias, out, M, N, K, epi, aux, aux_i, dtype, variant};
    g.out16 = out16; g.partials = partials; g.prow = prow; g.lead = lead;
    if (epi == VH_EPI_PATCH_SPLIT && aux_i > 0 && prow && prow < (M / aux_i) * (int64_t)(aux_i + lead))
        return fail(nullptr, VH_ERR_INVALID, "gemm_lead: prow is below images x (aux_i + lead)");
    return op_gemm_run("gemm_lead", g, 0, stream);
}
int vh_op_lead_rows(void* x_or_hi, void* lo, float* partials, int64_t prow, const float* cls, const float* pos, const float* reg, int lead,
                    int batch, int tokens, int dim, int dtype, void* stream) {
    const bool no_cls = !cls && !pos;
    if (!x_or_hi || (!no_cls && (!cls || !pos)) || batch <= 0 || dim <= 0 || dim % 64 || lead < 1 || lead > (no_cls ? 0 : 1) + VH_MAX_REGISTERS ||
        lead >= tokens || ((no_cls || lead > 1) && !reg))
        return fail(nullptr, VH_ERR_INVALID, "lead_rows: bad argument (dim %% 64 == 0, 1 <= lead <= 17, lead < tokens, reg for lead > 1)");
    hipError_t e;
    if (lo) {
        if (!partials || (dtype != VH_DTYPE_BF16 && dtype != VH_DTYPE_FP16) || prow < (int64_t)batch * tokens)
            return fail(nullptr, VH_ERR_INVALID, "lead_rows: the split form needs partials, a 16-bit dtype and prow >= batch x tokens");
        e = launch_lead_rows_split(x_or_hi, lo, partials, prow, cls, pos, reg, lead, batch, tokens, dim, dtype, (hipStream_t)stream);
    } else {
        e = launch_lead_rows((float*)x_or_hi, cls, pos, reg, lead, batch, tokens, dim, (hipStream_t)stream);
    }
    if (e == hipSuccess) e = hipStreamSynchronize((hipStream_t)stream);
    if (e != hipSuccess) return fail(nullptr, VH_ERR_HIP, "lead_rows failed: %s", hipGetErrorString(e));
    return VH_OK;
}
int vh_op_gemm_fp8(const void* a8, const void* w8, const float* w_scale, const float* bias, void* out, int64_t M, int N, int K,
                   int epi, int variant, void* stream) {
    GemmArgs g{a8, w8, bias, out, M, N, K, epi, nullptr, 0, VH_DTYPE_FP8, variant};
    g.wscale = w_scale;
    return op_gemm_run("gemm_fp8", g, kEpiPlain8, stream);
}
int vh_op_gemm_fp8_ex(const void* a8, const void* w8, const float* w_scale, const float* bias, void* out, int64_t M, int N, int K,
                      int epi, const float* c_dev, const float* stats, void* out16, float* partials, int variant, void* stream) {
    GemmArgs g{a8, w8, bias, out, M, N, K, epi, c_dev, 0, VH_DTYPE_FP8, variant};
    g.wscale = w_scale; g.stats = stats; g.out16 = out16; g.partials = partials;
    return op_gemm_run("gemm_fp8_ex", g, kEpiFold8, stream);
}
int vh_op_gemm_fp8_layout(const void* a8, const void* w8, const float* w_scale, const float* bias, void* out, int64_t M, int N, int K,
                          int epi, const float* c_dev, const float* stats, void* out16, float* partials, int variant,
                          int out_tiled, int ab_tiled, int tile_begin, int tile_count, void* stream) {
    GemmArgs g{a8, w8, bias, out, M, N, K, epi, c_dev, 0, VH_DTYPE_FP8, variant};
    g.wscale = w_scale; g.stats = stats; g.out16 = out16; g.partials = partials;
    g.out_tiled = out_tiled; g.ab_tiled = ab_tiled; g.tile_begin = tile_begin; g.tile_count = tile_count;
    return op_gemm_run("gemm_fp8_layout", g, kEpiPlain8 | kEpiFold8, stream);
}
int vh_op_quantize_rows(const float* w, int rows, int cols, float post_scale, void* w8, float* scale, void* stream) {
    if (!w || !w8 || !scale || rows <= 0 || cols <= 0 || cols % 4) return fail(nullptr, VH_ERR_INVALID, "quantize_rows: bad argument");
    OPCHK(launch_quantize_rows(w, rows, cols, post_scale, w8, scale, (hipStream_t)stream));
// ... 126 lines not shown
    OPCHK(hipStreamSynchronize((hipStream_t)stream));
    return VH_OK;
}
int vh_op_attention(const void* qkv16, int batch, int tokens, int heads, void* out16, int dtype, void* stream) {
    if (!qkv16 || !out16) return fail(nullptr, VH_ERR_INVALID, "null pointer");
    if (batch <= 0 || tokens <= 0 || heads <= 0 || tokens > kAttnStreamMaxTokens ||
        (attention_lds_bytes(tokens) > 160 * 1024 && heads > 32))
        return fail(nullptr, VH_ERR_INVALID, "attention: unsupported shape");
    unsigned int* ticket = nullptr;
    OPCHK(hipMalloc((void**)&ticket, 256));
    hipError_t e = launch_attention(qkv16, batch, tokens, heads, out16, dtype, ticket, (hipStream_t)stream);
    if (e == hipSuccess) e = hipStreamSynchronize((hipStream_t)stream);
    hipFree(ticket);
    if (e != hipSuccess) return fail(nullptr, VH_ERR_HIP, "attention failed: %s", hipGetErrorString(e));
    return VH_OK;
}
int vh_op_attention_stream(const void* qkv16, int batch, int tokens, int heads, void* out16, int dtype, void* stream) {
    if (!qkv16 || !out16) return fail(nullptr, VH_ERR_INVALID, "null pointer");
    if (batch <= 0 || tokens <= 0 || tokens > kAttnStreamMaxTokens || heads <= 0 || heads > 32)
        return fail(nullptr, VH_ERR_INVALID, "attention_stream: unsupported shape");
    if (dtype != VH_DTYPE_BF16 && dtype != VH_DTYPE_FP16 && dtype != VH_DTYPE_FP8)
        return fail(nullptr, VH_ERR_INVALID, "attention_stream: unsupported dtype");
    OPCHK(launch_attention_hd(qkv16, batch, tokens, heads, 64, out16, dtype, (hipStream_t)stream));
    OPCHK(hipStreamSynchronize((hipStream_t)stream));
    return VH_OK;
}
int vh_op_attention_hd(const void* qkv16, int batch, int tokens, int heads, int head_dim, void* out16, int dtype, void* stream) {
    if (!qkv16 || !out16) return fail(nullptr, VH_ERR_INVALID, "null pointer");
    if (!attention_hd_supported(head_dim)) return fail(nullptr, VH_ERR_INVALID, "attention_hd: head_dim must be 32, 48, ..., 128");
    if (batch <= 0 || tokens <= 0 || tokens > kAttnStreamMaxTokens || heads <= 0 || heads > kAttnHdMaxWidth / head_dim)
        return fail(nullptr, VH_ERR_INVALID, "attention_hd: unsupported shape");
    if (dtype != VH_DTYPE_BF16 && dtype != VH_DTYPE_FP16 && dtype != VH_DTYPE_FP8)
        return fail(nullptr, VH_ERR_INVALID, "attention_hd: unsupported dtype");
    OPCHK(launch_attention_hd(qkv16, batch, tokens, heads, head_dim, out16, dtype, (hipStream_t)stream));
    OPCHK(hipStreamSynchronize((hipStream_t)stream));
    return VH_OK;
}
int vh_op_attention_cls(const void* qkv16, int batch, int tokens, int heads, void* out16, int dtype, void* stream) {
    if (!qkv16 || !out16) return fail(nullptr, VH_ERR_INVALID, "null pointer");
    if (batch <= 0 || tokens <= 0 || tokens > 1024 || heads <= 0) return fail(nullptr, VH_ERR_INVALID, "attention_cls: unsupported shape");
    if (dtype != VH_DTYPE_BF16 && dtype != VH_DTYPE_FP16) return fail(nullptr, VH_ERR_INVALID, "attention_cls: unsupported dtype");
    OPCHK(launch_attention_cls(qkv16, batch, tokens, heads, out16, dtype, (hipStream_t)stream));
    OPCHK(hipStreamSynchronize((hipStream_t)stream));
    return VH_OK;
}
int vh_op_attention_layout(const void* qkv16, int batch, int tokens, int heads, void* out16, int dtype, int out_tiled, int64_t in_hm_rows,
                           void* stream) {
    if (!qkv16 || !out16) return fail(nullptr, VH_ERR_INVALID, "null pointer");
    if (batch <= 0 || tokens <= 0 || heads <= 0 || tokens > kAttnStreamMaxTokens ||
        (attention_lds_bytes(tokens) > 160 * 1024 && heads > 32))
        return fail(nullptr, VH_ERR_INVALID, "attention_layout: unsupported shape");
    if (dtype != VH_DTYPE_BF16 && dtype != VH_DTYPE_FP16 && dtype != VH_DTYPE_FP8)
        return fail(nullptr, VH_ERR_INVALID, "attention_layout: unsupported dtype");
    if (in_hm_rows < 0 || (in_hm_rows && !out_tiled)) return fail(nullptr, VH_ERR_INVALID, "attention_layout: head-major q|k|v needs the tiled output");
    if (in_hm_rows && (in_hm_rows < (int64_t)batch * tokens || in_hm_rows * heads * 64 * 4 >= (1ll << 32)))
        return fail(nullptr, VH_ERR_INVALID, "attention_layout: in_hm_rows must hold batch * tokens rows (and 4 * in_hm_rows * heads * 64 < 2^32)");
    if (out_tiled && !attention_tiled_applies(batch, tokens, heads))
        return fail(nullptr, VH_ERR_INVALID, "attention_layout: the tiled output exists in the ring forms with an even head count only");
    unsigned int* ticket = nullptr;
    OPCHK(hipMalloc((void**)&ticket, 256));
    hipError_t e = launch_attention(qkv16, batch, tokens, heads, out16, dtype, ticket, (hipStream_t)stream, false, out_tiled != 0, in_hm_rows);
    if (e == hipSuccess) e = hipStreamSynchronize((hipStream_t)stream);
    hipFree(ticket);
    if (e != hipSuccess) return fail(nullptr, e == hipErrorInvalidValue ? VH_ERR_INVALID : VH_ERR_HIP, "attention_layout failed: %s", hipGetErrorString(e));
    return VH_OK;
}
int vh_op_attention_probs(const void* qkv16, int batch, int tokens, int heads, int head_dim, int queries, int64_t in_hm_rows, int dtype,
                          float* probs, void* stream) {
    if (!qkv16 || !probs) return fail(nullptr, VH_ERR_INVALID, "attention_probs: null pointer");
    if (batch <= 0) return fail(nullptr, VH_ERR_INVALID, "attention_probs: batch %d must be positive", batch);
    if (tokens < 1 || tokens > kAttnStreamMaxTokens) return fail(nullptr, VH_ERR_INVALID, "attention_probs: tokens %d outside 1..%d", tokens, kAttnStreamMaxTokens);
    if (!attention_hd_supported(head_dim)) return fail(nullptr, VH_ERR_INVALID, "attention_probs: head_dim %d is not 32, 48, ..., 128", head_dim);
    if (heads <= 0 || heads > kAttnHdMaxWidth / head_dim)
        return fail(nullptr, VH_ERR_INVALID, "attention_probs: heads %d x head_dim %d outside 1..%d", heads, head_dim, kAttnHdMaxWidth);
    if (queries < 1 || queries > kAttnMapsMaxQueries || queries > tokens)
        return fail(nullptr, VH_ERR_INVALID, "attention_probs: queries %d outside 1..min(%d, tokens)", queries, kAttnMapsMaxQueries);
    if (dtype != VH_DTYPE_BF16 && dtype != VH_DTYPE_FP16) return fail(nullptr, VH_ERR_INVALID, "attention_probs: dtype %d is not VH_DTYPE_BF16 or VH_DTYPE_FP16", dtype);
    if (in_hm_rows && head_dim != 64) return fail(nullptr, VH_ERR_INVALID, "attention_probs: head-major q|k|v (in_hm_rows != 0) exists at head_dim 64 only, not %d", head_dim);
    if (in_hm_rows && in_hm_rows < (int64_t)batch * tokens)
        return fail(nullptr, VH_ERR_INVALID, "attention_probs: in_hm_rows %lld holds fewer than batch * tokens = %lld rows", (long long)in_hm_rows, (long long)batch * tokens);
    if (((uintptr_t)qkv16 | (uintptr_t)probs) & 15)
        return fail(nullptr, VH_ERR_INVALID, "attention_probs: a pointer is not 16-byte aligned (qkv16 %p, probs %p)", qkv16, (void*)probs);
    if (const char* why = attention_probs_check(in_hm_rows, batch, tokens, heads, head_dim, queries, dtype)) return fail(nullptr, VH_ERR_INVALID, "attention_probs: %s", why);
    OPCHK(launch_attention_probs(qkv16, in_hm_rows, batch, tokens, heads, head_dim, queries, dtype, probs, (hipStream_t)stream));
    OPCHK(hipStreamSynchronize((hipStream_t)stream));
    return VH_OK;
}
int vh_op_attention_readout(const float* store, int batch, int heads, int queries, int tokens, int lead, int elem, int keys, void* probs_out,
                            void* head_mean_out, void* stream) {
    if (!store) return fail(nullptr, VH_ERR_INVALID, "attention_readout: null store");
    if (!probs_out && !head_mean_out) return fail(nullptr, VH_ERR_INVALID, "attention_readout: no output requested (probs_out and head_mean_out are both NULL)");
    if (batch <= 0) return fail(nullptr, VH_ERR_INVALID, "attention_readout: batch %d must be positive", batch);
    if (heads <= 0 || heads > kAttnHdMaxWidth / 32) return fail(nullptr, VH_ERR_INVALID, "attention_readout: heads %d outside 1..%d", heads, kAttnHdMaxWidth / 32);
    if (tokens < 1 || tokens > kAttnStreamMaxTokens) return fail(nullptr, VH_ERR_INVALID, "attention_readout: tokens %d outside 1..%d", tokens, kAttnStreamMaxTokens);
    if (queries < 1 || queries > kAttnMapsMaxQueries || queries > tokens)
        return fail(nullptr, VH_ERR_INVALID, "attention_readout: queries %d outside 1..min(%d, tokens)", queries, kAttnMapsMaxQueries);
    if (lead < 0 || lead >= tokens) return fail(nullptr, VH_ERR_INVALID, "attention_readout: lead %d outside 0..tokens-1", lead);
    if (elem != VH_ELEM_F32 && elem != VH_ELEM_F16 && elem != VH_ELEM_BF16)
        return fail(nullptr, VH_ERR_INVALID, "attention_readout: elem %d is not VH_ELEM_F32, VH_ELEM_F16 or VH_ELEM_BF16", elem);
    if (keys != VH_ATTN_KEYS_ALL && keys != VH_ATTN_KEYS_PATCH)
        return fail(nullptr, VH_ERR_INVALID, "attention_readout: keys %d is not VH_ATTN_KEYS_ALL (0) or VH_ATTN_KEYS_PATCH (1)", keys);
    if (((uintptr_t)store | (uintptr_t)probs_out | (uintptr_t)head_mean_out) & 15)
        return fail(nullptr, VH_ERR_INVALID, "attention_readout: a pointer is not 16-byte aligned (store %p, probs_out %p, head_mean_out %p)", (const void*)store,
                    probs_out, head_mean_out);
    if (const char* why = attention_readout_check(batch, heads, queries, tokens, lead, elem, keys)) return fail(nullptr, VH_ERR_INVALID, "attention_readout: %s", why);
    OPCHK(launch_attention_readout(store, batch, heads, queries, tokens, lead, elem, keys, probs_out, head_mean_out, (hipStream_t)stream));
    OPCHK(hipStreamSynchronize((hipStream_t)stream));
    return VH_OK;
}
int vh_op_im2col(const float* in, int batch, int image, int patch, int channels, void* out16, int dtype, void* stream) {
    if (!in || !out16) return fail(nullptr, VH_ERR_INVALID, "null pointer");
    if (batch <= 0 || patch <= 0 || image <= 0 || image % patch || (patch * channels) % 4)
        return fail(nullptr, VH_ERR_INVALID, "im2col: unsupported shape");
    OPCHK(launch_im2col(in, batch, image, patch, channels, patch * patch * channels, out16, dtype, (hipStream_t)stream));
// ... 756 lines not shown
```

vit-fpga_amd/python/vithip.py:

```python
from __future__ import annotations

import ctypes as C
import os

import numpy as np

_HERE = os.path.dirname(os.path.abspath(__file__))
PKG_ROOT = os.path.dirname(_HERE)
REPO_ROOT = os.path.dirname(PKG_ROOT)
LIB_PATH = os.environ.get("VITHIP_LIB") or os.path.join(PKG_ROOT, "libvithip.so")

DTYPE_BF16, DTYPE_FP16, DTYPE_FP8 = 0, 1, 2
FLAG_LN_FOLD_OFF, FLAG_LN_FOLD_ON, FLAG_W8_E4M3, FLAG_CLS_TAIL = 1, 2, 4, 8
FLAG_PRE_LN, FLAG_QUICK_GELU = 16, 32
FLAG_REGISTERS_MASK, MAX_REGISTERS = 31 << 9, 16


def FLAG_REGISTERS(n):
    return (int(n) & 31) << 9


def registers_of(flags):
    return (int(flags) & FLAG_REGISTERS_MASK) >> 9

# ... 908 lines not shown
        if px.dtype != dtype or px.ndim != 3 or px.shape[2] != 3 or px.size == 0:
            raise TypeError(f"pack_frames_bgra: frame {i} is not [H, W, 3] {np.dtype(dtype).name} samples (or three [H, W] planes)")
        h, w = px.shape[:2]
        pos = [(lay >> (2 * k)) & 3 for k in range(3)]
        if lay & 256:
            if dtype != np.uint16 or lay not in (L444_Y410, L444_V410):
                raise ValueError(f"pack_frames_bgra: frame {i}: a 10-bit layout is L444_Y410 or L444_V410 and takes uint16 codes")
            rows = _sample_bytes(word10_rows(px[..., 0], px[..., 1], px[..., 2], lay))
        else:
            ns = 4 if lay & 64 else 3
            if lay < 0 or lay > 255 or max(pos) >= ns:
                raise ValueError(f"pack_frames_bgra: frame {i}: layout {lay} is no VH_444 word")
            m = np.full((h, w, ns), np.iinfo(dtype).max, dtype)
            for k in range(3):
                m[:, :, pos[k]] = px[..., k]
            rows = _sample_bytes(m)
        d = desc[i]
        d.offset, d.height, d.width, d.row_stride, d.layout = off, h, w, rows.size // h, lay
        d.box[:] = (0.0, 0.0, float(w), float(h)) if box is None else tuple(float(b) for b in box)
        parts.append(rows)
        off += rows.size
    return np.concatenate(parts), desc


def make_config(cfg, dtype=DTYPE_BF16, max_batch=1, ln_eps=1e-6, flags=0):
    r = int(cfg.get("registers", 0))
    if not 0 <= r <= 31:
        raise ValueError(f"make_config: cfg['registers'] = {r} is outside 0 .. 31 (the library takes 0 .. {MAX_REGISTERS})")
    if r and registers_of(flags) not in (0, r):
        raise ValueError(f"make_config: cfg['registers'] = {r} but flags carry FLAG_REGISTERS({registers_of(flags)})")
    flags |= FLAG_REGISTERS(r)
    return Config(cfg["image_size"], cfg["patch_size"], cfg["channels"], cfg["dim"], cfg["heads"],
                  cfg["mlp_dim"], cfg["layers"], cfg["classes"], dtype, max_batch, ln_eps, flags)


def to_bf16_bits(a):
    u = np.ascontiguousarray(a, dtype=np.float32).view(np.uint32)
    r = u + np.uint32(0x7FFF) + ((u >> np.uint32(16)) & np.uint32(1))
    return (r >> np.uint32(16)).astype(np.uint16)


def from_bf16_bits(b):
    return (np.ascontiguousarray(b, dtype=np.uint16).astype(np.uint32) << np.uint32(16)).view(np.float32)


def to16(a, dtype):
    return to_bf16_bits(a) if dtype == DTYPE_BF16 else np.ascontiguousarray(a, dtype=np.float16).view(np.uint16)


def from16(b, dtype):
    return from_bf16_bits(b) if dtype == DTYPE_BF16 else np.ascontiguousarray(b, dtype=np.uint16).view(np.float16).astype(np.float32)


def pack_head_major(qkv, heads, hm_rows, fill=0):
    qkv = np.ascontiguousarray(qkv)
    rows = qkv.shape[0]
    assert qkv.shape[1] == 3 * heads * 64 and hm_rows >= rows
    out = np.full((3, heads, hm_rows, 64), fill, dtype=qkv.dtype)
    out[:, :, :rows] = qkv.reshape(rows, 3, heads, 64).transpose(1, 2, 0, 3)
    return out


def unpack_tiled(tiled, rows, dim, chunk=8):
    nb = (rows + 15) // 16
    t = np.ascontiguousarray(tiled).reshape(nb, dim // chunk, 16, chunk)
    return np.ascontiguousarray(t.transpose(0, 2, 1, 3).reshape(nb * 16, dim)[:rows])


def pack_tiled(a, chunk=8, fill=0):
    a = np.ascontiguousarray(a)
    rows, dim = a.shape
    assert dim % chunk == 0
    nb = (rows + 15) // 16
    full = np.full((nb * 16, dim), fill, dtype=a.dtype)
    full[:rows] = a
    return np.ascontiguousarray(full.reshape(nb, 16, dim // chunk, chunk).transpose(0, 2, 1, 3))


_NUMPY_ELEM = {np.dtype(np.float32): ELEM_F32, np.dtype(np.float16): ELEM_F16, np.dtype(np.uint8): ELEM_U8}


class DeviceBuffer:

    def __init__(self, nbytes, device=0):
        self.device, self.nbytes = device, int(nbytes)
        p = C.c_void_p()
        _check(lib().vh_malloc(device, self.nbytes, C.byref(p)))
        self.ptr = p.value

    @classmethod
    def from_numpy(cls, a, device=0):
        a = np.ascontiguousarray(a)
        b = cls(a.nbytes, device)
        _check(lib().vh_memcpy_h2d(device, b.ptr, a.ctypes.data, a.nbytes))
        return b

    def to_numpy(self, dtype, shape):
        out = np.empty(shape, dtype=dtype)
        assert out.nbytes <= self.nbytes
        _check(lib().vh_memcpy_d2h(self.device, out.ctypes.data, self.ptr, out.nbytes))
        return out

    def free(self):
        if self.ptr:
            lib().vh_free(self.device, self.ptr)
            self.ptr = None

    def __del__(self):
        try:
            self.free()
        except Exception:
            pass
# ... 796 lines not shown


def op_quantize_rows(w_ptr, rows, cols, post_scale, w8_ptr, scale_ptr):
    _check(lib().vh_op_quantize_rows(w_ptr, rows, cols, post_scale, w8_ptr, scale_ptr, None))


def op_gemm_fp8_ex(a8_ptr, w8_ptr, scale_ptr, bias_ptr, out_ptr, M, N, K, epilogue, c_ptr=None, stats_ptr=None, out16_ptr=None,
                   partials_ptr=None, variant=0):
    _check(lib().vh_op_gemm_fp8_ex(a8_ptr, w8_ptr, scale_ptr, bias_ptr, out_ptr, M, N, K, epilogue, c_ptr, stats_ptr, out16_ptr,
                                   partials_ptr, variant, None))


def e4m3_table():
    b = np.arange(256, dtype=np.uint32)
    e, m = (b >> 3) & 15, b & 7
    v = np.where(e == 0, m * 2.0 ** -9, (1 + m / 8.0) * 2.0 ** (e.astype(np.float64) - 7))
    v = np.where((e == 15) & (m == 7), np.nan, v)
    return np.where(b >> 7 == 1, -v, v).astype(np.float32)


def from_e4m3(b):
    return e4m3_table()[np.ascontiguousarray(b, dtype=np.uint8)]


def to_e4m3(x):
    x = np.ascontiguousarray(x, dtype=np.float32)
    pos = e4m3_table()[:127].astype(np.float64)
    a = np.minimum(np.abs(x).astype(np.float64), 448.0)
    hi = np.clip(np.searchsorted(pos, a, side="left"), 1, 126)
    lo = hi - 1
    dl, dh = a - pos[lo], pos[hi] - a
    code = np.where(dl < dh, lo, np.where(dh < dl, hi, np.where(lo % 2 == 0, lo, hi)))
    return (code | np.where(np.signbit(x), 0x80, 0)).astype(np.uint8)


LO8_SCALE = {DTYPE_BF16: 32.0, DTYPE_FP16: 256.0}


def to_lo8(residue, dtype):
    return to_e4m3(np.asarray(residue, dtype=np.float32) * np.float32(LO8_SCALE[dtype]))


def from_lo8(b, dtype):
    return from_e4m3(b) / np.float32(LO8_SCALE[dtype])


def op_gemm_ex(a_ptr, w_ptr, bias_ptr, out_ptr, M, N, K, epilogue, dtype, aux_ptr=None, aux_i=0, stats_ptr=None,
               out16_ptr=None, partials_ptr=None, variant=0):
    _check(lib().vh_op_gemm_ex(a_ptr, w_ptr, bias_ptr, out_ptr, M, N, K, epilogue, aux_ptr, aux_i, stats_ptr, out16_ptr,
                               partials_ptr, dtype, variant, None))


def op_gemm_layout(a_ptr, w_ptr, bias_ptr, out_ptr, M, N, K, epilogue, dtype, aux_ptr=None, aux_i=0, stats_ptr=None,
                   out16_ptr=None, partials_ptr=None, variant=0, out_tiled=False, ab_tiled=False, tile_begin=0, tile_count=0):
    _check(lib().vh_op_gemm_layout(a_ptr, w_ptr, bias_ptr, out_ptr, M, N, K, epilogue, aux_ptr, aux_i, stats_ptr, out16_ptr,
                                   partials_ptr, dtype, variant, 1 if out_tiled else 0, 1 if ab_tiled else 0, tile_begin, tile_count, None))


def op_gemm_lead(a_ptr, w_ptr, bias_ptr, out_ptr, M, N, K, epilogue, dtype, pos_ptr, patches, lead, out16_ptr=None, partials_ptr=None,
                 prow=0, variant=0):
    _check(lib().vh_op_gemm_lead(a_ptr, w_ptr, bias_ptr, out_ptr, M, N, K, epilogue, pos_ptr, patches, lead, out16_ptr, partials_ptr,
                                 prow, dtype, variant, None))


def op_lead_rows(x_or_hi_ptr, cls_ptr, pos_ptr, reg_ptr, lead, batch, tokens, dim, lo_ptr=None, partials_ptr=None, prow=0,
                 dtype=DTYPE_BF16):
    _check(lib().vh_op_lead_rows(x_or_hi_ptr, lo_ptr, partials_ptr, prow, cls_ptr, pos_ptr, reg_ptr, lead, batch, tokens, dim, dtype, None))


def op_gemm_fp8_layout(a8_ptr, w8_ptr, scale_ptr, bias_ptr, out_ptr, M, N, K, epilogue, c_ptr=None, stats_ptr=None, out16_ptr=None,
                       partials_ptr=None, variant=0, out_tiled=False, ab_tiled=False, tile_begin=0, tile_count=0):
    _check(lib().vh_op_gemm_fp8_layout(a8_ptr, w8_ptr, scale_ptr, bias_ptr, out_ptr, M, N, K, epilogue, c_ptr, stats_ptr, out16_ptr,
                                       partials_ptr, variant, 1 if out_tiled else 0, 1 if ab_tiled else 0, tile_begin, tile_count, None))


def op_tile_rows(in_ptr, rows, cols, out_ptr, dtype):
    _check(lib().vh_op_tile_rows(in_ptr, rows, cols, out_ptr, dtype, None))


def op_rowstats_cast(x_ptr, rows, dim, eps, x16_ptr, stats_ptr, dtype):
    _check(lib().vh_op_rowstats_cast(x_ptr, rows, dim, eps, x16_ptr, stats_ptr, dtype, None))


def op_rowstats_split(x_ptr, rows, dim, eps, hi_ptr, lo_ptr, stats_ptr, dtype):
    _check(lib().vh_op_rowstats_split(x_ptr, rows, dim, eps, hi_ptr, lo_ptr, stats_ptr, dtype, None))


def op_pre_layernorm(x_ptr, rows, dim, gamma_ptr, beta_ptr, eps, y32_ptr, hi_ptr, lo_ptr, stats_ptr, dtype):
    _check(lib().vh_op_pre_layernorm(x_ptr, rows, dim, gamma_ptr, beta_ptr, eps, y32_ptr, hi_ptr, lo_ptr, stats_ptr, dtype, None))


def op_finalize_stats(partials_ptr, nblk, rows, dim, eps, stats_ptr):
    _check(lib().vh_op_finalize_stats(partials_ptr, nblk, rows, dim, eps, stats_ptr, None))


def op_fold_ln(w_ptr, b_ptr, gamma_ptr, beta_ptr, rows, dim, scale, w16_ptr, c_ptr, d_ptr, dtype):
    _check(lib().vh_op_fold_ln(w_ptr, b_ptr, gamma_ptr, beta_ptr, rows, dim, scale, w16_ptr, c_ptr, d_ptr, dtype, None))


def op_rowstats_guard(x_ptr, rows, dim, eps, hi_ptr, lo_ptr, stats_ptr, dtype, guard_rows=0, amax_guard_ptr=None):
    _check(lib().vh_op_rowstats_guard(x_ptr, rows, dim, eps, hi_ptr, lo_ptr, stats_ptr, dtype, guard_rows, amax_guard_ptr, None))


def op_pre_layernorm_guard(x_ptr, rows, dim, gamma_ptr, beta_ptr, eps, y32_ptr, hi_ptr, lo_ptr, stats_ptr, dtype, guard_rows=0,
                           guard_ptr=None, amax_guard_ptr=None):
    _check(lib().vh_op_pre_layernorm_guard(x_ptr, rows, dim, gamma_ptr, beta_ptr, eps, y32_ptr, hi_ptr, lo_ptr, stats_ptr, dtype,
                                           guard_rows, guard_ptr, amax_guard_ptr, None))


# ... 23 lines not shown

def op_fake_quant_rows(w_ptr, rows, cols, out_ptr):
    _check(lib().vh_op_fake_quant_rows(w_ptr, rows, cols, out_ptr, None))


def bench_gemm(M, N, K, epilogue, dtype=DTYPE_BF16, variant=0, iters=20, device=0):
    ms = C.c_double(0)
    _check(lib().vh_bench_gemm(device, M, N, K, epilogue, dtype, variant, iters, C.byref(ms)))
    return ms.value


def op_token_features(hi_ptr, lo_ptr, form, batch, tokens, dim, gamma_ptr, beta_ptr, eps, elem, norm, patch_ptr, mean_ptr):
    _check(lib().vh_op_token_features(hi_ptr, lo_ptr, form, batch, tokens, dim, gamma_ptr, beta_ptr, eps, elem, norm, patch_ptr, mean_ptr, None))


def op_token_features2(hi_ptr, lo_ptr, form, batch, tokens, lead, dim, gamma_ptr, beta_ptr, eps, elem, norm, patch_ptr, patch_layout,
                       mean_ptr, reg_ptr):
    _check(lib().vh_op_token_features2(hi_ptr, lo_ptr, form, batch, tokens, lead, dim, gamma_ptr, beta_ptr, eps, elem, norm, patch_ptr,
                                       patch_layout, mean_ptr, reg_ptr, None))


def op_pool_rows(hi_ptr, lo_ptr, form, batch, tokens, lead, dim, gamma_ptr, beta_ptr, eps, norm, mean_ptr):
    _check(lib().vh_op_pool_rows(hi_ptr, lo_ptr, form, batch, tokens, lead, dim, gamma_ptr, beta_ptr, eps, norm, mean_ptr, None))


def op_map_pool(hi_ptr, lo_ptr, form, batch, tokens, lead, dim, gamma_ptr, beta_ptr, eps, qk_ptr, heads, z_ptr):
    _check(lib().vh_op_map_pool(hi_ptr, lo_ptr, form, batch, tokens, lead, dim, gamma_ptr, beta_ptr, eps, qk_ptr, heads, z_ptr, None))


def op_rope(qkv_ptr, dtype, batch, tokens, heads, head_dim, lead, hm_rows, cos_ptr, sin_ptr):
    _check(lib().vh_op_rope(qkv_ptr, dtype, batch, tokens, heads, head_dim, lead, hm_rows, cos_ptr, sin_ptr, None))


def op_layernorm(x_ptr, rows, dim, row_stride, gamma_ptr, beta_ptr, eps, out_ptr, dtype):
    _check(lib().vh_op_layernorm(x_ptr, rows, dim, row_stride, gamma_ptr, beta_ptr, eps, out_ptr, dtype, None))


def op_attention(qkv_ptr, batch, tokens, heads, out_ptr, dtype):
    _check(lib().vh_op_attention(qkv_ptr, batch, tokens, heads, out_ptr, dtype, None))


def op_attention_stream(qkv_ptr, batch, tokens, heads, out_ptr, dtype):
    _check(lib().vh_op_attention_stream(qkv_ptr, batch, tokens, heads, out_ptr, dtype, None))


def op_attention_hd(qkv_ptr, batch, tokens, heads, head_dim, out_ptr, dtype):
    _check(lib().vh_op_attention_hd(qkv_ptr, batch, tokens, heads, head_dim, out_ptr, dtype, None))


def op_attention_cls(qkv_ptr, batch, tokens, heads, out_ptr, dtype):
    _check(lib().vh_op_attention_cls(qkv_ptr, batch, tokens, heads, out_ptr, dtype, None))


def op_attention_layout(qkv_ptr, batch, tokens, heads, out_ptr, dtype, out_tiled=False, in_hm_rows=0):
    _check(lib().vh_op_attention_layout(qkv_ptr, batch, tokens, heads, out_ptr, dtype, 1 if out_tiled else 0, in_hm_rows, None))


def op_attention_probs(qkv_ptr, batch, tokens, heads, head_dim, queries, dtype, probs_ptr, in_hm_rows=0):
    _check(lib().vh_op_attention_probs(qkv_ptr, batch, tokens, heads, head_dim, queries, in_hm_rows, dtype, probs_ptr, None))


def op_attention_readout(store_ptr, batch, heads, queries, tokens, lead, elem, keys, probs_ptr, head_mean_ptr):
    _check(lib().vh_op_attention_readout(store_ptr, batch, heads, queries, tokens, lead, elem, keys, probs_ptr, head_mean_ptr, None))


def op_im2col(in_ptr, batch, image, patch, channels, out_ptr, dtype):
    _check(lib().vh_op_im2col(in_ptr, batch, image, patch, channels, out_ptr, dtype, None))


def op_im2col_padded(in_ptr, batch, image, patch, channels, kpad, out_ptr, dtype):
    _check(lib().vh_op_im2col_padded(in_ptr, batch, image, patch, channels, kpad, out_ptr, dtype, None))


def op_im2col_u8(in_ptr, batch, image, patch, channels, kpad, scale, shift, out_ptr, dtype):
    sc = None if scale is None else np.ascontiguousarray(scale, dtype=np.float32).reshape(-1)
    sh = None if shift is None else np.ascontiguousarray(shift, dtype=np.float32).reshape(-1)
    for a in (sc, sh):
        if a is not None and a.size != channels:
            raise ValueError(f"op_im2col_u8: expected {channels} values per array, got {a.size}")
    _check(lib().vh_op_im2col_u8(in_ptr, batch, image, patch, channels, kpad, None if sc is None else sc.ctypes.data,
                                 None if sh is None else sh.ctypes.data, out_ptr, dtype, None))


def op_im2col_tensor(in_ptr, elem, layout, batch, image, patch, channels, kpad, out_ptr, dtype, scale=None, shift=None):
    sc = None if scale is None else np.ascontiguousarray(scale, dtype=np.float32).reshape(-1)
    sh = None if shift is None else np.ascontiguousarray(shift, dtype=np.float32).reshape(-1)
    for a in (sc, sh):
        if a is not None and a.size != channels:
            raise ValueError(f"op_im2col_tensor: expected {channels} values per array, got {a.size}")
    _check(lib().vh_op_im2col_tensor(in_ptr, elem, layout, batch, image, patch, channels, kpad, None if sc is None else sc.ctypes.data,
                                     None if sh is None else sh.ctypes.data, out_ptr, dtype, None))


def op_resize_u8(frames_ptr, nbytes, desc, channels, out_size, out_ptr):
    _check(lib().vh_op_resize_u8(frames_ptr, nbytes, C.addressof(desc), len(desc), channels, out_size, out_ptr, None))


def _op_resize_colour(name, fn, frames_ptr, nbytes, desc, out_size, m, chroma_site, out_ptr):
    m = np.ascontiguousarray(m, dtype=np.float32).reshape(-1)
    if m.size != 12:
        raise ValueError(f"{name}: expected 12 matrix entries, got {m.size}")
    _check(fn(frames_ptr, nbytes, C.addressof(desc), len(desc), out_size, m.ctypes.data, chroma_site, out_ptr, None))


def op_resize_yuv(frames_ptr, nbytes, desc, out_size, m, chroma_site, out_ptr):
    _op_resize_colour("op_resize_yuv", lib().vh_op_resize_yuv, frames_ptr, nbytes, desc, out_size, m, chroma_site, out_ptr)


# ... 35 lines not shown
```

Before: 29130 images/s.

## Write Q and K head-major planes in 16-row blocked layout for attention

Adds a blocked output mode to the QKV GEMM epilogue. The Q and K planes are stored in 16-row blocks, using permlane16 swaps to form 16-byte stores, while V stays row-major. The attention ring kernel gains a matching input mode that DMAs and reads Q and K fragments straight from the blocked layout, with no XOR swizzle, and can use a smaller Q LDS region. The aim is to make the GEMM stores and the attention K/Q loads contiguous and cheaper. The cost is a new layout path with more kernel variants and stricter shape constraints. It is enabled by default through the VH_QKV_BLK environment variable.

Result: no change. 29170 images/s (median of 6 runs) (+0.1%).

```diff
diff --git a/vit-fpga_amd/csrc/gemm_epilogue.h b/vit-fpga_amd/csrc/gemm_epilogue.h
--- a/vit-fpga_amd/csrc/gemm_epilogue.h
+++ b/vit-fpga_amd/csrc/gemm_epilogue.h
@@ -29,13 +29,16 @@
     int lead;
 };
 
+constexpr int kEpiBlocked = 0x40;
+constexpr int epi_base(int epi) { return epi & ~kEpiBlocked; }
+constexpr bool epi_blocked(int epi) { return (epi & kEpiBlocked) != 0; }
 constexpr bool epi_has_qgelu(int epi) { return epi == VH_EPI_BIAS_QGELU || epi == VH_EPI_LNFOLD_QGELU; }
 constexpr bool epi_has_tgelu(int epi) { return epi == VH_EPI_BIAS_TGELU || epi == VH_EPI_LNFOLD_TGELU; }
 constexpr bool epi_has_act(int epi) { return epi == VH_EPI_BIAS_GELU || epi == VH_EPI_LNFOLD_GELU || epi_has_qgelu(epi) || epi_has_tgelu(epi); }
 constexpr bool epi_is_lnfold(int epi) {
-    return epi == VH_EPI_LNFOLD || epi == VH_EPI_LNFOLD_GELU || epi == VH_EPI_LNFOLD_QGELU || epi == VH_EPI_LNFOLD_TGELU;
-}
-constexpr bool epi_is_16bit(int epi) { return epi == VH_EPI_BIAS || epi == VH_EPI_LNFOLD || epi_has_act(epi); }
+    return epi_base(epi) == VH_EPI_LNFOLD || epi == VH_EPI_LNFOLD_GELU || epi == VH_EPI_LNFOLD_QGELU || epi == VH_EPI_LNFOLD_TGELU;
+}
+constexpr bool epi_is_16bit(int epi) { return epi_base(epi) == VH_EPI_BIAS || epi_base(epi) == VH_EPI_LNFOLD || epi_has_act(epi); }
 
 __device__ __forceinline__ float gelu_fast(float v) {
     const float u = fabsf(v);
@@ -257,6 +260,36 @@
         else consts_from_global();
     } else {
         consts_from_global();
+    }
+
+    if constexpr (epi_blocked(EPI)) {
+        static_assert(epi_is_16bit(EPI) && !epi_has_act(EPI) && MFULL && OTILED, "blocked q|k|v: LNFOLD / BIAS, whole tiles");
+        if (n_w < (((N >> 6) * 2) / 3) << 6) {
+            char* const obase = (char*)e.out + ((int64_t)(n_w >> 6) * M * 8 + (int64_t)(m_w >> 4) * 128 + (fq & 1) * 32 + (fq >> 1) * 16 + frow) * 16;
+#pragma unroll
+            for (int mi = 0; mi < MI; ++mi) {
+                if constexpr (VH_EPI_PRIO == 1) {
+                    if (prio_grp >= 0 && (mi & 1) == 0) {
+                        if (((mi >> 1) + prio_grp) & 1) __builtin_amdgcn_s_setprio(1);
+                        else __builtin_amdgcn_s_setprio(0);
+                    }
+                }
+                float rstd = 0.f, mr = 0.f;
+                if constexpr (epi_is_lnfold(EPI)) { rstd = lnst[mi].y; mr = lnst[mi].x * lnst[mi].y; }
+#pragma unroll
+                for (int j = 0; j < NI / 2; ++j) {
+                    const f32x4 v0 = epi_value16<EPI, T>(acc[mi][2 * j], bv[2 * j], cv[2 * j], mr, rstd);
+                    const f32x4 v1 = epi_value16<EPI, T>(acc[mi][2 * j + 1], bv[2 * j + 1], cv[2 * j + 1], mr, rstd);
+                    const u32x2 p0 = __builtin_bit_cast(u32x2, pack4<T>(v0[0], v0[1], v0[2], v0[3]));
+                    const u32x2 p1 = __builtin_bit_cast(u32x2, pack4<T>(v1[0], v1[1], v1[2], v1[3]));
+                    const auto sx = __builtin_amdgcn_permlane16_swap(p0[0], p1[0], false, false);
+                    const auto sy = __builtin_amdgcn_permlane16_swap(p0[1], p1[1], false, false);
+                    epi_store(u32x4{sx[0], sy[0], sx[1], sy[1]}, (u32x4*)(obase + mi * 2048 + j * 1024));
+                }
+            }
+            if constexpr (VH_EPI_PRIO == 1) { if (prio_grp >= 0) __builtin_amdgcn_s_setprio(0); }
+            return;
+        }
     }
 
     if constexpr (epi_is_16bit(EPI) && (VH_EPI_ABL & 64)) {
diff --git a/vit-fpga_amd/csrc/kernels_attn.hip b/vit-fpga_amd/csrc/kernels_attn.hip
--- a/vit-fpga_amd/csrc/kernels_attn.hip
+++ b/vit-fpga_amd/csrc/kernels_attn.hip
@@ -192,7 +192,7 @@
     asm volatile("s_waitcnt vmcnt(0)" ::: "memory");
 }
 
-template <typename T, typename TO = T, bool QS = false, bool OTILE = false, bool IHM = false>
+template <typename T, typename TO = T, bool QS = false, bool OTILE = false, bool IHM = false, bool IBK = false>
 __global__ void __launch_bounds__(1024, 4)
 attention_ring_kernel(const typename T::elem* __restrict__ qkv, typename TO::elem* __restrict__ out,
                       int tokens, int heads, int slabs, int ntiles, int nitems, unsigned int* __restrict__ ticket,
@@ -201,8 +201,10 @@
     using vec8 = typename T::vec8;
     using vec4 = typename T::vec4;
     extern __shared__ __attribute__((aligned(16))) char smem[];
+    static_assert(!IBK || (IHM && std::is_same<T, TO>::value), "blocked q and k: head-major planes, 16-bit results");
     const int G = (tokens + 7) >> 3, G2 = (G + 1) & ~1;
-    const int kv_bytes = QS ? G * 1024 : ntiles * 4096;
+    const int GK = IBK ? 2 * ((tokens + 15) >> 4) : G;
+    const int kv_bytes = QS ? GK * 1024 : ntiles * 4096;
     const int q_off = kv_bytes + (QS ? G2 * 1024 : kv_bytes);
     const uint32_t lds0 = (uint32_t)(uintptr_t)smem;
 
@@ -211,6 +213,7 @@
     const int nw = blockDim.x >> 6;
     const int l31 = lane & 31, hl = lane >> 5;
     const int D = heads * 64;
+    const int QP = IBK && GK < 4 * nw ? GK : 4 * nw;
     const int64_t ld = IHM ? 64 : 3 * (int64_t)D;
     const uint32_t koff2 = IHM ? (uint32_t)(hm_rows * D * 2) : (uint32_t)(D * 2);
     auto head_base = [&](int b, int h) {
@@ -227,17 +230,33 @@
         const int b = bh / heads, h = bh - b * heads;
         return head_base(b, h);
     };
+    auto blk_row0 = [&](const elem*& base) {
+        const int o = (int)((base - qkv) >> 6) & 15;
+        base -= o * 64;
+        return o;
+    };
+    auto blk_piece_off = [&](int p, int ln, int o) {
+        const int row = (p >> 1) * 16 + (ln & 15);
+        const int r = (row < tokens ? row : tokens - 1) + o;
+        return (uint32_t)((r >> 4) * 2048 + ((p & 1) * 4 + (ln >> 4)) * 256 + (r & 15) * 16);
+    };
     auto issue_tile = [&](const elem* base, int t) {
         int ln = lane;
         asm volatile("" : "+v"(ln));
         const int lr_ = ln >> 3, pc_ = ln & 7;
         const int g = 4 * t + wave;
-        const int gk = QS && g >= G ? G - 1 : g, gv = QS && g >= G2 ? G2 - 1 : g;
+        const int gk = QS && g >= GK ? GK - 1 : g, gv = QS && g >= G2 ? G2 - 1 : g;
         const int rowk = gk * 8 + lr_, rowv = gv * 8 + lr_;
         const int rk = rowk < tokens ? rowk : tokens - 1;
         const int rv = rowv < tokens ? rowv : tokens - 1;
         const int ck = pc_ ^ ((rowk >> 1) & 7);
         const int cv = pc_ ^ (((rowv >> 1) & 1) << 2);
+        if constexpr (IBK) {
+            const int o = blk_row0(base);
+            ring_dma16(base, blk_piece_off(gk, ln, o) + koff2, lds0 + gk * 1024);
+            ring_dma16(base, (uint32_t)((rv + o) * 64 + cv * 8) * 2u + 2u * koff2, lds0 + kv_bytes + gv * 1024);
+            return;
+        }
         const uint32_t ok = (uint32_t)(rk * (int)ld + ck * 8) * 2u + koff2;
         const uint32_t ov = (uint32_t)(rv * (int)ld + cv * 8) * 2u + 2u * koff2;
         ring_dma16(base, ok, lds0 + gk * 1024);
@@ -247,6 +266,14 @@
         int ln = lane;
         asm volatile("" : "+v"(ln));
         const int lr_ = ln >> 3, pc_ = ln & 7;
+        if constexpr (IBK) {
+            const int o = blk_row0(base);
+            for (int j = 0; j < nw; ++j) {
+                const int g = 4 * j + wave, gq = g >= QP ? QP - 1 : g;
+                ring_dma16(base, blk_piece_off(gq, ln, o), lds0 + q_off + gq * 1024);
+            }
+            return;
+        }
         for (int j = 0; j < nw; ++j) {
             const int g = 4 * j + wave;
             const int row = g * 8 + lr_;
@@ -260,6 +287,15 @@
         const int b = bh / heads, h = bh - b * heads;
         int qrow = (slab * nw + wave) * 32 + l31;
         qrow = qrow < tokens ? qrow : tokens - 1;
+        if constexpr (IBK) {
+            const elem* base = head_base(b, h);
+            const int r = blk_row0(base) + qrow;
+            const elem* qp = base + ((r >> 4) * 1024 + (r & 15) * 8 + 128 * hl);
+            asm volatile("global_load_dwordx4 %0, %4, off\n\tglobal_load_dwordx4 %1, %4, off offset:512\n\t"
+                         "global_load_dwordx4 %2, %4, off offset:1024\n\tglobal_load_dwordx4 %3, %4, off offset:1536"
+                         : "=&v"(qf[0]), "=&v"(qf[1]), "=&v"(qf[2]), "=&v"(qf[3]) : "v"(qp) : "memory");
+            return;
+        }
         const elem* qp = head_base(b, h) + (int64_t)qrow * ld + 8 * hl;
         asm volatile("global_load_dwordx4 %0, %4, off\n\tglobal_load_dwordx4 %1, %4, off offset:32\n\t"
                      "global_load_dwordx4 %2, %4, off offset:64\n\tglobal_load_dwordx4 %3, %4, off offset:96"
@@ -270,7 +306,8 @@
     const int g4 = lane >> 4, i16 = lane & 15, tq = i16 >> 2, tp = i16 & 3;
     const int vrow0 = 4 * (g4 >> 1) + tq;
     const int vcolb = (16 * (g4 & 1) + 4 * tp) * 2;
-    const int k0 = l31 * 128 + ((hl ^ kswz) << 4);
+    const int k0 = IBK ? (l31 >> 4) * 2048 + hl * 256 + (l31 & 15) * 16
+                       : l31 * 128 + ((hl ^ kswz) << 4);
     const int vx = ((vrow0 >> 1) & 1) << 6;
     const int v0 = kv_bytes + vrow0 * 128 + (vcolb ^ vx);
 
@@ -295,7 +332,7 @@
     unsigned long long ph_[10] = {0, 0, 0, 0, 0, 0, 0, 0, 0, 0}, last_ = attn_ct();
 #endif
     const bool dyn = QS && ticket != nullptr && nw >= 5;
-    const int tk_off = q_off + 4 * nw * 1024;
+    const int tk_off = q_off + QP * 1024;
     unsigned int tkv = 0;
     while (true) {
         const int slab_now = QS ? 0 : item - (item / slabs) * slabs;
@@ -344,8 +381,18 @@
                 const int r31 = ln & 31;
                 qa = q_off + wave * 4096 + r31 * 128 + ((((ln >> 5)) ^ ((r31 >> 1) & 7)) << 4);
             }
+            if constexpr (IBK) {
+                int ln = lane;
+                asm volatile("" : "+v"(ln));
+                int row = wave * 32 + (ln & 31);
+                row = row < QP * 8 ? row : QP * 8 - 1;
+                qa = q_off + (row >> 4) * 2048 + (ln >> 5) * 256 + (row & 15) * 16;
+#pragma unroll
+                for (int ks = 0; ks < 4; ++ks) qf[ks] = *(const vec8*)(smem + (qa + (ks << 9)));
+            } else {
 #pragma unroll
             for (int ks = 0; ks < 4; ++ks) qf[ks] = *(const vec8*)(smem + (qa ^ (ks << 5)));
+            }
         }
 
         f32x16 o0, o1;
@@ -361,7 +408,7 @@
 #pragma unroll
             for (int ks = 0; ks < 4; ++ks) {
                 if (VH_ATTN_ABL & 32) kf[ks] = qf[ks]; else if (VH_ATTN_ABL & 128) kf[ks] = *(const vec8*)(smem + ((ka ^ (ks << 5)) & 0x3ff0)); else
-                kf[ks] = *(const vec8*)(smem + (ka ^ (ks << 5)));
+                kf[ks] = *(const vec8*)(smem + (IBK ? ka + (ks << 9) : ka ^ (ks << 5)));
             }
             __builtin_amdgcn_sched_barrier(0);
             typedef float f32x2 __attribute__((ext_vector_type(2)));
@@ -564,14 +611,15 @@
 
 enum class AttnForm { NONE, ONE_SHOT, RING, RING_QS };
 struct AttnPlan { AttnForm form; int slabs, nw; size_t lds; };
-static AttnPlan attn_plan(int tokens, bool out_tiled, bool in_head_major) {
+static AttnPlan attn_plan(int tokens, bool out_tiled, bool in_head_major, bool in_blocked = false) {
     constexpr int kMaxWaves = 16;
     const int ntiles = (tokens + 31) / 32;
     const int slabs = (ntiles + kMaxWaves - 1) / kMaxWaves, nw = (ntiles + slabs - 1) / slabs;
     const size_t one = attention_lds_bytes(tokens);
     if (one > 160 * 1024) return {AttnForm::NONE, slabs, nw, 0};
     const int G = (tokens + 7) / 8, G2 = (G + 1) & ~1;
-    const size_t qs_lds = (size_t)(G + G2 + 4 * nw) * 1024 + 16;
+    const int GK = in_blocked ? 2 * ((tokens + 15) / 16) : G, QP = in_blocked && GK < 4 * nw ? GK : 4 * nw;
+    const size_t qs_lds = (size_t)(GK + G2 + QP) * 1024 + 16;
     if (slabs == 1 && nw >= 4 && 2 * qs_lds <= 160 * 1024) return {AttnForm::RING_QS, slabs, nw, qs_lds};
     if (ntiles >= 3 && nw >= 4) return {AttnForm::RING, slabs, nw, one};
     if (out_tiled || in_head_major) return {AttnForm::NONE, slabs, nw, 0};
@@ -582,17 +630,19 @@
     return attn_plan(tokens, true, false).form != AttnForm::NONE && heads % 2 == 0;
 }
 
-template <typename T, typename TO = T, bool OTILE = false, bool IHM = false>
+bool attention_ring_applies(int tokens) { return attn_plan(tokens, true, true).form != AttnForm::NONE; }
+
+template <typename T, typename TO = T, bool OTILE = false, bool IHM = false, bool IBK = false>
 static hipError_t launch_attn_t(const void* qkv, int batch, int tokens, int heads, void* out, unsigned int* ticket, hipStream_t s, bool tk_zeroed,
                                 int64_t hm_rows = 0) {
-    const AttnPlan p = attn_plan(tokens, OTILE, IHM);
+    const AttnPlan p = attn_plan(tokens, OTILE, IHM, IBK);
     if (p.form == AttnForm::NONE) return hipErrorInvalidValue;
     const int ntiles = (tokens + 31) / 32, slabs = p.slabs, nw = p.nw;
     const int nitems = batch * heads * slabs;
     const int num_cu = device_num_cu();
     if (!num_cu) return hipErrorUnknown;
     if (p.form == AttnForm::RING_QS) {
-        auto k = attention_ring_kernel<T, TO, true, OTILE, IHM>;
+        auto k = attention_ring_kernel<T, TO, true, OTILE, IHM, IBK>;
         static LdsDone lds_done;
         if (hipError_t e = ensure_dynamic_lds((const void*)k, p.lds, lds_done); e != hipSuccess) return e;
         const int grid = nitems < 2 * num_cu ? nitems : 2 * num_cu;
@@ -604,7 +654,7 @@
         return hipGetLastError();
     }
     if (p.form == AttnForm::RING) {
-        auto k = attention_ring_kernel<T, TO, false, OTILE, IHM>;
+        auto k = attention_ring_kernel<T, TO, false, OTILE, IHM, IBK>;
         static LdsDone lds_done;
         if (hipError_t e = ensure_dynamic_lds((const void*)k, p.lds, lds_done); e != hipSuccess) return e;
         const int per_cu = (int)(160 * 1024 / p.lds);
@@ -721,11 +771,17 @@
 }
 
 hipError_t launch_attention(const void* qkv16, int batch, int tokens, int heads, void* out16, int dtype,
-                            unsigned int* ticket, hipStream_t s, bool ticket_zeroed, bool out_tiled, int64_t in_hm_rows) {
+                            unsigned int* ticket, hipStream_t s, bool ticket_zeroed, bool out_tiled, int64_t in_hm_rows, bool in_blocked) {
     if (batch <= 0 || tokens <= 0 || heads <= 0) return hipErrorInvalidValue;
+    if (in_blocked) {
+        if (!in_hm_rows || !out_tiled || in_hm_rows % 16 || in_hm_rows < (int64_t)batch * tokens || in_hm_rows * heads * 64 * 4 >= (1ll << 32)) return hipErrorInvalidValue;
+        if (!attention_ring_applies(tokens) || (dtype != VH_DTYPE_BF16 && dtype != VH_DTYPE_FP16)) return hipErrorInvalidValue;
+        return dtype == VH_DTYPE_BF16 ? launch_attn_t<BF16, BF16, true, true, true>(qkv16, batch, tokens, heads, out16, ticket, s, ticket_zeroed, in_hm_rows)
+                                      : launch_attn_t<FP16, FP16, true, true, true>(qkv16, batch, tokens, heads, out16, ticket, s, ticket_zeroed, in_hm_rows);
+    }
     if (in_hm_rows) {
         if (!out_tiled || in_hm_rows < (int64_t)batch * tokens || in_hm_rows * heads * 64 * 4 >= (1ll << 32)) return hipErrorInvalidValue;
-        if (!attention_tiled_applies(batch, tokens, heads)) return hipErrorInvalidValue;
+        if (!attention_ring_applies(tokens)) return hipErrorInvalidValue;
         if (dtype == VH_DTYPE_FP8) return launch_attn_t<BF16, E4M3, true, true>(qkv16, batch, tokens, heads, out16, ticket, s, ticket_zeroed, in_hm_rows);
         return dtype == VH_DTYPE_BF16 ? launch_attn_t<BF16, BF16, true, true>(qkv16, batch, tokens, heads, out16, ticket, s, ticket_zeroed, in_hm_rows)
                                       : launch_attn_t<FP16, FP16, true, true>(qkv16, batch, tokens, heads, out16, ticket, s, ticket_zeroed, in_hm_rows);
diff --git a/vit-fpga_amd/csrc/kernels_gemm.hip b/vit-fpga_amd/csrc/kernels_gemm.hip
--- a/vit-fpga_amd/csrc/kernels_gemm.hip
+++ b/vit-fpga_amd/csrc/kernels_gemm.hip
@@ -210,6 +210,8 @@
                         : "gemm_layout: the tiled layouts need at least 2 K-tiles with this epilogue";
         if (g.out_tiled && !(act || epi == VH_EPI_LNFOLD || (!f8 && epi == VH_EPI_BIAS)))
             return "gemm_layout: out_tiled goes with the activation epilogues (tiled) or LNFOLD / 16-bit BIAS (head-major)";
+        if (g.out_blocked && !(g.out_tiled && !f8 && (epi == VH_EPI_LNFOLD || epi == VH_EPI_BIAS)))
+            return "gemm_layout: out_blocked goes with out_tiled and 16-bit LNFOLD / BIAS (q|k|v)";
         if (g.ab_tiled && !(epi == VH_EPI_RESID_SPLIT || (!f8 && epi == VH_EPI_BIAS))) return "gemm_layout: ab_tiled goes with RESID_SPLIT or 16-bit BIAS";
     }
     if (g.tile_begin < 0 || g.tile_count < 0) return "gemm_layout: negative tile range";
diff --git a/vit-fpga_amd/csrc/kernels_gemm5.hip b/vit-fpga_amd/csrc/kernels_gemm5.hip
--- a/vit-fpga_amd/csrc/kernels_gemm5.hip
+++ b/vit-fpga_amd/csrc/kernels_gemm5.hip
@@ -488,6 +488,9 @@
             const int num_cu = device_num_cu();
             if (!num_cu) return hipErrorUnknown;
             const int nfull = full_m * tiles_n, grid = nfull < num_cu ? nfull : num_cu;
+            if constexpr (!F8 && (EPI == VH_EPI_LNFOLD || EPI == VH_EPI_BIAS)) {
+                if (g.out_tiled && g.out_blocked) return launch_pp_one<T, EPI | kEpiBlocked, F8, true, 2, true, false>(g, grid, full_m, tiles_n, s);
+            }
             if constexpr (epi_has_act(EPI) || EPI == VH_EPI_LNFOLD || (!F8 && EPI == VH_EPI_BIAS)) {
                 if (g.out_tiled) return launch_pp_one<T, EPI, F8, true, 2, true, false>(g, grid, full_m, tiles_n, s);
             }
diff --git a/vit-fpga_amd/csrc/vh_kernels.h b/vit-fpga_amd/csrc/vh_kernels.h
--- a/vit-fpga_amd/csrc/vh_kernels.h
+++ b/vit-fpga_amd/csrc/vh_kernels.h
@@ -27,6 +27,7 @@
     int tile_begin = 0, tile_count = 0;
     int64_t prow = 0;
     int out_tiled = 0, ab_tiled = 0;
+    int out_blocked = 0;
     int lead = 1;
 };
 bool gemm_tiled_applies(int64_t M, int N, int K, int dtype);
@@ -54,8 +55,10 @@
 constexpr float kAttnQScale = 0.125f * 1.4426950408889634f;
 hipError_t launch_attention(const void* qkv16, int batch, int tokens, int heads, void* out16,
                             int dtype, unsigned int* ticket, hipStream_t stream, bool ticket_zeroed = false, bool out_tiled = false,
-                            int64_t in_hm_rows = 0);
+                            int64_t in_hm_rows = 0,
+                            bool in_blocked = false);
 bool attention_tiled_applies(int batch, int tokens, int heads);
+bool attention_ring_applies(int tokens);
 hipError_t launch_attention_cls(const void* qkv16, int batch, int tokens, int heads, void* out16, int dtype, hipStream_t stream);
 size_t attention_lds_bytes(int tokens);
 constexpr int kAttnStreamMaxTokens = 4097;
diff --git a/vit-fpga_amd/csrc/vithip_api.hip b/vit-fpga_amd/csrc/vithip_api.hip
--- a/vit-fpga_amd/csrc/vithip_api.hip
+++ b/vit-fpga_amd/csrc/vithip_api.hip
@@ -240,6 +240,7 @@
     bool h_tiled = false;
     bool att_tiled = true;
     bool qkv_hm = true;
+    bool qkv_blk = true;
     bool weights_ready_tiled = false;
     float* bqkv = nullptr;
     bool fp8 = false;
@@ -302,6 +303,7 @@
     int ring_batch = 0, ring_wr = 0, ring_rd = 0, ring_used = 0;
     bool last_h_tiled = false;
     bool last_qkv_hm = false;
+    bool last_qkv_blk = false;
     int num_cu = 256;
     bool use_graph = false;
     struct GraphEntry { ImgIn in; float* out; int batch; hipGraph_t graph; hipGraphExec_t exec; };
@@ -641,9 +643,11 @@
                       (size_t)L.NP * L.KPA * esz >= 2 * ((size_t)D * esz + 256);
     const bool h_tiled = c->h_tiled && c->split && c->weights_ready_tiled && gemm_tiled_applies(rows_g, M, D, op_dt) && gemm_tiled_applies(rows_g, D, M, op_dt);
     const bool att_tiled = hd64 && h_tiled && c->att_tiled && gemm_tiled_applies(rows_g, D, D, op_dt) && attention_tiled_applies(batch, T, f.heads) && !tail;
-    const bool qkv_hm = c->qkv_hm && att_tiled && gemm_tiled_applies(rows_g, 3 * D, D, op_dt);
+    const bool qkv_hm = c->qkv_hm && att_tiled && gemm_tiled_applies(rows_g, 3 * D, D, op_dt) && (int64_t)rows_g * D * 4 < (1ll << 32);
+    const bool qkv_blk = qkv_hm && c->qkv_blk && !c->fp8 && hd64 && !L.rope && !c->attn_store && c->attn_n == 0 && !tail;
     c->last_h_tiled = h_tiled && nl > 0 && c->ln_fold;
     c->last_qkv_hm = qkv_hm && nl > 0 && c->ln_fold;
+    c->last_qkv_blk = qkv_blk && nl > 0 && c->ln_fold;
     for (int l = 0; l < nl && c->ln_fold; ++l) {
         const LayerOff& o = L.layer[l];
         const float* cd = c->fold_cd + (size_t)l * (6 * D + 2 * M);
@@ -653,6 +657,7 @@
         GemmArgs gq = gemm_args(op_dt, xn16, c->wqkv16[l], cd + 3 * D, qkv16, rows_g, 3 * D, D, VH_EPI_LNFOLD, cd);
         gq.wscale = sq;
         set_tiled(gq, qkv_hm, false);
+        gq.out_blocked = qkv_blk;
         if ((rc = stage(ST_QKV, [&] { return launch_gemm(gq, s); }))) return rc;
         if ((rc = rope(qkv_hm ? (int64_t)rows_g : 0))) return rc;
         if ((rc = capture_attention(l, qkv_hm ? (int64_t)rows_g : 0))) return rc;
@@ -685,7 +690,7 @@
             return VH_OK;
         }
         if ((rc = stage(ST_ATTN, [&] {
-                 return hd64 ? launch_attention(qkv16, batch, T, f.heads, att16, op_dt, tickets_part + l, s, true, att_tiled, qkv_hm ? (int64_t)rows_g : 0)
+                 return hd64 ? launch_attention(qkv16, batch, T, f.heads, att16, op_dt, tickets_part + l, s, true, att_tiled, qkv_hm ? (int64_t)rows_g : 0, qkv_blk)
                              : launch_attention_hd(qkv16, batch, T, f.heads, c->head_dim, att16, op_dt, s);
              })))
             return rc;
@@ -1322,6 +1327,7 @@
         c->h_tiled = want_tiled || want_tiled8;
         { const char* e = getenv("VH_ATT_TILED"); c->att_tiled = !(e && e[0] == '0'); }
         { const char* e = getenv("VH_QKV_HM"); c->qkv_hm = !(e && e[0] == '0'); }
+        { const char* e = getenv("VH_QKV_BLK"); c->qkv_blk = !(e && e[0] == '0'); }
     }
     CK(hipHostMalloc((void**)&c->guard_host, 64, hipHostMallocDefault));
     *c->guard_host = 0.f;
@@ -2260,6 +2266,11 @@
         host_out[0] = c->last_qkv_hm ? 1.f : 0.f;
         return VH_OK;
     }
+    if (what == 5) {
+        if (n_floats != 1) return fail(&c->err, VH_ERR_INVALID, "expected 1 float");
+        host_out[0] = c->last_qkv_blk ? 1.f : 0.f;
+        return VH_OK;
+    }
     return fail(&c->err, VH_ERR_INVALID, "unknown tap %d", what);
 }
 
@@ -2630,7 +2641,7 @@
                       int out_tiled, int ab_tiled, int tile_begin, int tile_count, void* stream) {
     GemmArgs g{a, w, bias, out, M, N, K, epi, aux, aux_i, dtype, variant};
     g.stats = stats; g.out16 = out16; g.partials = partials;
-    g.out_tiled = out_tiled; g.ab_tiled = ab_tiled; g.tile_begin = tile_begin; g.tile_count = tile_count;
+    g.out_tiled = out_tiled != 0; g.out_blocked = out_tiled == 2; g.ab_tiled = ab_tiled; g.tile_begin = tile_begin; g.tile_count = tile_count;
     return op_gemm_run("gemm_layout", g, 0, stream);
 }
 int vh_op_gemm_lead(const void* a, const void* w, const float* bias, void* out, int64_t M, int N, int K, int epi, const float* aux,
@@ -2863,14 +2874,19 @@
         return fail(nullptr, VH_ERR_INVALID, "attention_layout: unsupported shape");
     if (dtype != VH_DTYPE_BF16 && dtype != VH_DTYPE_FP16 && dtype != VH_DTYPE_FP8)
         return fail(nullptr, VH_ERR_INVALID, "attention_layout: unsupported dtype");
+    const bool in_blocked = out_tiled == 3;
+    if (in_blocked && (!in_hm_rows || in_hm_rows % 16 || dtype == VH_DTYPE_FP8))
+        return fail(nullptr, VH_ERR_INVALID, "attention_layout: blocked q and k need head-major planes of in_hm_rows %% 16 == 0 rows and a 16-bit dtype");
     if (in_hm_rows < 0 || (in_hm_rows && !out_tiled)) return fail(nullptr, VH_ERR_INVALID, "attention_layout: head-major q|k|v needs the tiled output");
     if (in_hm_rows && (in_hm_rows < (int64_t)batch * tokens || in_hm_rows * heads * 64 * 4 >= (1ll << 32)))
         return fail(nullptr, VH_ERR_INVALID, "attention_layout: in_hm_rows must hold batch * tokens rows (and 4 * in_hm_rows * heads * 64 < 2^32)");
-    if (out_tiled && !attention_tiled_applies(batch, tokens, heads))
+    if (out_tiled && in_hm_rows && !attention_ring_applies(tokens))
+        return fail(nullptr, VH_ERR_INVALID, "attention_layout: head-major q|k|v exists in the ring forms only");
+    if (out_tiled && !in_hm_rows && !attention_tiled_applies(batch, tokens, heads))
         return fail(nullptr, VH_ERR_INVALID, "attention_layout: the tiled output exists in the ring forms with an even head count only");
     unsigned int* ticket = nullptr;
     OPCHK(hipMalloc((void**)&ticket, 256));
-    hipError_t e = launch_attention(qkv16, batch, tokens, heads, out16, dtype, ticket, (hipStream_t)stream, false, out_tiled != 0, in_hm_rows);
+    hipError_t e = launch_attention(qkv16, batch, tokens, heads, out16, dtype, ticket, (hipStream_t)stream, false, out_tiled != 0, in_hm_rows, in_blocked);
     if (e == hipSuccess) e = hipStreamSynchronize((hipStream_t)stream);
     hipFree(ticket);
     if (e != hipSuccess) return fail(nullptr, e == hipErrorInvalidValue ? VH_ERR_INVALID : VH_ERR_HIP, "attention_layout failed: %s", hipGetErrorString(e));
diff --git a/vit-fpga_amd/python/vithip.py b/vit-fpga_amd/python/vithip.py
--- a/vit-fpga_amd/python/vithip.py
+++ b/vit-fpga_amd/python/vithip.py
@@ -984,12 +984,31 @@
     return from_bf16_bits(b) if dtype == DTYPE_BF16 else np.ascontiguousarray(b, dtype=np.uint16).view(np.float16).astype(np.float32)
 
 
-def pack_head_major(qkv, heads, hm_rows, fill=0):
+def pack_head_major(qkv, heads, hm_rows, fill=0, blocked=False):
     qkv = np.ascontiguousarray(qkv)
     rows = qkv.shape[0]
     assert qkv.shape[1] == 3 * heads * 64 and hm_rows >= rows
     out = np.full((3, heads, hm_rows, 64), fill, dtype=qkv.dtype)
     out[:, :, :rows] = qkv.reshape(rows, 3, heads, 64).transpose(1, 2, 0, 3)
+    if blocked:
+        out = block_planes(out.reshape(3 * heads, hm_rows, 64)).reshape(3, heads, hm_rows, 64)
+    return out
+
+
+def blocked_planes(n_planes):
+    return n_planes * 2 // 3
+
+
+def block_planes(planes, inverse=False):
+    planes = np.ascontiguousarray(planes)
+    P, rows, w = planes.shape
+    assert w == 64 and rows % 16 == 0 and planes.dtype.itemsize == 2
+    out = planes.copy()
+    nb = blocked_planes(P)
+    if inverse:
+        out[:nb] = planes[:nb].reshape(nb, rows // 16, 8, 16, 8).transpose(0, 1, 3, 2, 4).reshape(nb, rows, 64)
+    else:
+        out[:nb] = planes[:nb].reshape(nb, rows // 16, 16, 8, 8).transpose(0, 1, 3, 2, 4).reshape(nb, rows, 64)
     return out
 
 
@@ -1892,9 +1911,11 @@
 
 
 def op_gemm_layout(a_ptr, w_ptr, bias_ptr, out_ptr, M, N, K, epilogue, dtype, aux_ptr=None, aux_i=0, stats_ptr=None,
-                   out16_ptr=None, partials_ptr=None, variant=0, out_tiled=False, ab_tiled=False, tile_begin=0, tile_count=0):
+                   out16_ptr=None, partials_ptr=None, variant=0, out_tiled=False, ab_tiled=False, tile_begin=0, tile_count=0,
+                   out_blocked=False):
     _check(lib().vh_op_gemm_layout(a_ptr, w_ptr, bias_ptr, out_ptr, M, N, K, epilogue, aux_ptr, aux_i, stats_ptr, out16_ptr,
-                                   partials_ptr, dtype, variant, 1 if out_tiled else 0, 1 if ab_tiled else 0, tile_begin, tile_count, None))
+                                   partials_ptr, dtype, variant, (2 if out_blocked else 1) if out_tiled else 0, 1 if ab_tiled else 0,
+                                   tile_begin, tile_count, None))
 
 
 def op_gemm_lead(a_ptr, w_ptr, bias_ptr, out_ptr, M, N, K, epilogue, dtype, pos_ptr, patches, lead, out16_ptr=None, partials_ptr=None,
@@ -2024,8 +2045,9 @@
     _check(lib().vh_op_attention_cls(qkv_ptr, batch, tokens, heads, out_ptr, dtype, None))
 
 
-def op_attention_layout(qkv_ptr, batch, tokens, heads, out_ptr, dtype, out_tiled=False, in_hm_rows=0):
-    _check(lib().vh_op_attention_layout(qkv_ptr, batch, tokens, heads, out_ptr, dtype, 1 if out_tiled else 0, in_hm_rows, None))
+def op_attention_layout(qkv_ptr, batch, tokens, heads, out_ptr, dtype, out_tiled=False, in_hm_rows=0, in_blocked=False):
+    _check(lib().vh_op_attention_layout(qkv_ptr, batch, tokens, heads, out_ptr, dtype, (3 if in_blocked else 1) if out_tiled else 0,
+                                        in_hm_rows, None))
 
 
 def op_attention_probs(qkv_ptr, batch, tokens, heads, head_dim, queries, dtype, probs_ptr, in_hm_rows=0):
```
